# JaronTu/Multimodal_MVD_Seg

Hardware: AMD Instinct MI355X
Metric: train-step samples/sec on 4-modality 128^3 patches (PlainConvUNet 3d_fullres, fp32) (higher is better)
Workload: dtype f32; 1 GPU; BASELINE configs[1]: PlainConvUNet 3d_fullres 6 stages 31.2M params, 4x128x128x128 patch, 5 classes, fp32, DC+CE deep supervision, SGD-Nesterov+clip; per_gpu_batch=2, global_batch=2, parallelism=dp1, step_launch=one hipGraph replay per step (captured after 3 eager steps)

## Files before the change

include/mvdseg_hip.h:

```cpp
#ifndef MVDSEG_HIP_H
#define MVDSEG_HIP_H
#include <stddef.h>
#include <stdint.h>

#ifdef __cplusplus
extern "C" {
#endif

#define MVD_VERSION 100
#define MVD_MAX_TAPS 27

int mvd_version(void);
const char *mvd_last_error(void);
int mvd_has_mfma(void);
int mvd_set_conv_engine(int mode);
int mvd_set_wino_min_items(long n);

int mvd_pack_weight(const float *w, float *wf, float *wb, int K, int C, int T, int transposed, void *stream);

size_t mvd_conv_fwd_workspace_bytes(int N, long out_voxels, int K);
int mvd_conv3d_fwd(const float *x1, int C1, const float *x2, int C2, const float *wf, const float *bias, float *y,
                   int N, int D, int H, int W, int K, const int ksize[3], const int stride[3], void *ws,
                   size_t ws_bytes, void *stream);
int mvd_conv3d_dgrad(const float *dy, const float *wb, float *dx1, int C1, float *dx2, int C2, int N, int D, int H,
                     int W, int K, const int ksize[3], const int stride[3], void *ws, size_t ws_bytes, void *stream);
int mvd_conv_wino_applicable(int N, int D, int H, int W, int C1, int C2, int K, const int ksize[3], const int stride[3]);
size_t mvd_wino_weight_elems(int C, int K);
int mvd_wino_mode(void);
int mvd_pack_weight_wino(const float *w, float *uf, float *ub, int K, int C, void *stream);
int mvd_pack_weights_batch(int n, const float *const *w, float *const *wf, float *const *wb, float *const *uf,
                           float *const *ub, const int *K, const int *C, const int *T, const int *transposed,
                           void *stream);
int mvd_conv3d_fwd_wino(const float *x1, int C1, const float *x2, int C2, const float *wf, const float *uf,
                        const float *bias, float *y, int N, int D, int H, int W, int K, const int ksize[3],
                        const int stride[3], void *ws, size_t ws_bytes, void *stream);
size_t mvd_conv_stats_tiles(int D, int H, int W);
int mvd_conv3d_fwd_wino_stats(const float *x1, int C1, const float *x2, int C2, const float *wf, const float *uf,
                              const float *bias, float *y, float *stats, int *stats_done, int N, int D, int H, int W,
                              int K, const int ksize[3], const int stride[3], void *ws, size_t ws_bytes, void *stream);
int mvd_conv3d_dgrad_wino(const float *dy, const float *wb, const float *ub, float *dx1, int C1, float *dx2, int C2, int N,
                          int D, int H, int W, int K, const int ksize[3], const int stride[3], void *ws, size_t ws_bytes,
                          void *stream);
int mvd_set_wino3_min_items(long n);
int mvd_conv_wino3_applicable(int N, int D, int H, int W, int C1, int C2, int K, const int ksize[3], const int stride[3]);
size_t mvd_wino3_weight_elems(int C, int K);
int mvd_pack_weight_wino3(const float *w, float *vf, float *vb, int K, int C, void *stream);
int mvd_pack_weights_batch3(int n, const float *const *w, float *const *wf, float *const *wb, float *const *uf,
                            float *const *ub, float *const *vf, float *const *vb, const int *K, const int *C,
                            const int *T, const int *transposed, void *stream);
int mvd_conv3d_fwd_wino3(const float *x1, int C1, const float *x2, int C2, const float *wf, const float *vf,
                         const float *bias, float *y, int N, int D, int H, int W, int K, const int ksize[3],
                         const int stride[3], void *ws, size_t ws_bytes, void *stream);
int mvd_conv3d_fwd_wino3_stats(const float *x1, int C1, const float *x2, int C2, const float *wf, const float *vf,
                               const float *bias, float *y, float *stats, int *stats_done, int N, int D, int H, int W,
                               int K, const int ksize[3], const int stride[3], void *ws, size_t ws_bytes, void *stream);
int mvd_conv3d_dgrad_wino3(const float *dy, const float *wb, const float *vb, float *dx1, int C1, float *dx2, int C2,
                           int N, int D, int H, int W, int K, const int ksize[3], const int stride[3], void *ws,
                           size_t ws_bytes, void *stream);
int mvd_set_wgrad_wino3_min_items(long n);
int mvd_conv_wgrad_wino3_applicable(int N, int D, int H, int W, int C1, int C2, int K, const int ksize[3],
                                    const int stride[3]);
long mvd_wgrad_wino3_launches(void);
size_t mvd_conv3d_wgrad_workspace_bytes(int C, int K, int T, int N, int Do, int Ho, int Wo);
int mvd_conv3d_wgrad(const float *x1, int C1, const float *x2, int C2, const float *dy, float *dw, float *dbias,
                     int N, int D, int H, int W, int K, const int ksize[3], const int stride[3], void *ws,
                     size_t ws_bytes, void *stream);

int mvd_convT3d_fwd(const float *x, const float *wf, const float *bias, float *y, int N, int D, int H, int W, int C,
                    int K, const int stride[3], void *ws, size_t ws_bytes, void *stream);
int mvd_convT3d_dgrad(const float *dy, const float *wb, float *dx, int N, int D, int H, int W, int C, int K,
                      const int stride[3], void *ws, size_t ws_bytes, void *stream);
size_t mvd_convT3d_wgrad_workspace_bytes(int C, int K, int T, int N, int D, int H, int W);
int mvd_convT3d_wgrad(const float *x, const float *dy, float *dw, float *dbias, int N, int D, int H, int W, int C,
                      int K, const int stride[3], void *ws, size_t ws_bytes, void *stream);

int mvd_pack_weight_bf16(const float *w, uint16_t *wf, uint16_t *wb, int K, int C, int T, int transposed, void *stream);
int mvd_pack_weights_bf16_batch(int n, const float *const *w, uint16_t *const *wf, uint16_t *const *wb, const int *K,
                                const int *C, const int *T, const int *transposed, void *stream);
int mvd_pack_weights_bf16_batch_pad(int n, const float *const *w, uint16_t *const *wf, uint16_t *const *wb, const int *K,
                                    const int *C, const int *T, const int *transposed, const int *Csrc, void *stream);
int mvd_conv3d_fwd_bf16(const uint16_t *x1, int C1, const uint16_t *x2, int C2, const uint16_t *wf, const float *bias,
                        uint16_t *y, int N, int D, int H, int W, int K, const int ksize[3], const int stride[3],
                        void *ws, size_t ws_bytes, void *stream);
int mvd_conv3d_dgrad_bf16(const uint16_t *dy, const uint16_t *wb, uint16_t *dx1, int C1, uint16_t *dx2, int C2, int N,
                          int D, int H, int W, int K, const int ksize[3], const int stride[3], void *ws, size_t ws_bytes,
                          void *stream);
int mvd_convT3d_fwd_bf16(const uint16_t *x, const uint16_t *wf, const float *bias, uint16_t *y, int N, int D, int H, int W,
                         int C, int K, const int stride[3], void *ws, size_t ws_bytes, void *stream);
int mvd_convT3d_dgrad_bf16(const uint16_t *dy, const uint16_t *wb, uint16_t *dx, int N, int D, int H, int W, int C, int K,
                           const int stride[3], void *ws, size_t ws_bytes, void *stream);
int mvd_conv3d_wgrad_bf16(const uint16_t *x1, int C1, const uint16_t *x2, int C2, const uint16_t *dy, float *dw,
                          float *dbias, int N, int D, int H, int W, int K, const int ksize[3], const int stride[3],
                          void *ws, size_t ws_bytes, void *stream);
int mvd_convT3d_wgrad_bf16(const uint16_t *x, const uint16_t *dy, float *dw, float *dbias, int N, int D, int H, int W,
                           int C, int K, const int stride[3], void *ws, size_t ws_bytes, void *stream);
int mvd_conv3d_fwd_bf16_stats_tiles(int N, int D, int H, int W, int C1, int C2, int K, const int ksize[3],
                                    const int stride[3]);
int mvd_conv3d_dgrad_acc_ok(int is_bf16, int N, int D, int H, int W, int C1, int K, const int ksize[3], const int stride[3]);
int mvd_conv3d_dgrad_acc(const float *dy, const float *wb, float *dx1, int C1, int N, int D, int H, int W, int K,
                         const int ksize[3], const int stride[3], void *stream);
int mvd_conv3d_dgrad_bf16_acc(const uint16_t *dy, const uint16_t *wb, uint16_t *dx1, int C1, int N, int D, int H, int W, int K,
                              const int ksize[3], const int stride[3], void *ws, size_t ws_bytes, void *stream);
int mvd_set_bf16_zmarch_kernel(int which);
int mvd_set_bf16_wgrad_kernel(int which);
int mvd_conv3d_wgrad_bf16_prologue_ok(int N, int D, int H, int W, int C1, int C2, int K, const int ksize[3], const int stride[3]);
int mvd_conv3d_wgrad_bf16_fused(const uint16_t *x1, int C1, const uint16_t *dy, float *dw, float *dbias, int N, int D, int H, int W,
                                int K, const int ksize[3], const int stride[3], const float *in_scale, const float *in_shift,
                                float slope, void *ws, size_t ws_bytes, void *stream);
int mvd_conv3d_fwd_bf16_prologue_ok(int N, int D, int H, int W, int C1, int C2, int K, const int ksize[3],
                                    const int stride[3]);
int mvd_conv3d_fwd_bf16_fused(const uint16_t *x1, int C1, const uint16_t *x2, int C2, const uint16_t *wf, const float *bias,
                              uint16_t *y, int N, int D, int H, int W, int K, const int ksize[3], const int stride[3],
                              const float *in_scale, const float *in_shift, float slope, float *tile_stats, int *ntiles_out,
                              void *ws, size_t ws_bytes, void *stream);
int mvd_instnorm_finalize_tiles(const float *tile_stats, long ntiles, const float *gamma, const float *beta, float *mean,
                                float *rstd, float *scale, float *shift, int N, long V, int C, float eps, void *stream);
int mvd_instnorm_lrelu_apply_bf16(const uint16_t *x, const float *scale, const float *shift, uint16_t *y, int N, long V,
                                  int C, float slope, void *stream);
int mvd_instnorm_stats_bf16(const void *x, int x_is_bf16, const float *gamma, const float *beta, float *mean, float *rstd,
                            float *scale, float *shift, int N, long V, int C, float eps, void *ws, size_t ws_bytes,
                            void *stream);
int mvd_instnorm_lrelu_fwd_bf16(const void *x, int x_is_bf16, const float *gamma, const float *beta, uint16_t *y,
                                float *mean, float *rstd, int N, long V, int C, float eps, float slope, void *ws,
                                size_t ws_bytes, void *stream);
int mvd_instnorm_lrelu_bwd_bf16(const void *x, int x_is_bf16, const uint16_t *dy, const float *gamma, const float *beta,
                                const float *mean, const float *rstd, void *dx, float *dgamma, float *dbeta, int N,
                                long V, int C, float slope, void *ws, size_t ws_bytes, void *stream);
int mvd_seghead_fwd_bf16(const uint16_t *x, const float *w, const float *bias, float *logits, int N, long V, int C,
                         int K, void *stream);
int mvd_seghead_bwd_bf16(const uint16_t *x, const float *w, const float *dlogits, uint16_t *dx, float *dw, float *dbias,
                         int N, long V, int C, int K, int accumulate, void *ws, size_t ws_bytes, void *stream);
int mvd_seghead_bf16_fused_ok(int N, long V, int C, int K);
int mvd_seghead_fwd_fused(const float *x, const float *mean, const float *rstd, const float *gamma, const float *beta, float slope,
                          const float *w, const float *bias, float *logits, int N, long V, int C, int K, void *stream);
int mvd_seghead_bwd_fused(const float *x, const float *mean, const float *rstd, const float *gamma, const float *beta, float slope,
                          const float *w, const float *dlogits, float *dx, float *dw, float *dbias, int N, long V, int C, int K,
                          int accumulate, void *ws, size_t ws_bytes, void *stream);
int mvd_instnorm_stats_from_tiles(const float *tile_stats, long ntiles, float *mean, float *rstd, int N, long V, int C, float eps,
                                  void *ws, size_t ws_bytes, void *stream);
int mvd_seghead_fwd_bf16_fused(const uint16_t *x, const float *scale, const float *shift, float slope, const float *w,
                               const float *bias, float *logits, int N, long V, int C, int K, void *stream);
int mvd_seghead_bwd_bf16_fused(const uint16_t *x, const float *scale, const float *shift, float slope, const float *w,
                               const float *dlogits, uint16_t *dx, float *dw, float *dbias, int N, long V, int C, int K,
                               int accumulate, void *ws, size_t ws_bytes, void *stream);
int mvd_cast_f32_to_bf16(const float *src, uint16_t *dst, long n, void *stream);
int mvd_cast_bf16_to_f32(const uint16_t *src, float *dst, long n, void *stream);

int mvd_instnorm_nblk(int N, long V, int C);
size_t mvd_instnorm_workspace_bytes(int N, long V, int C);
int mvd_instnorm_lrelu_fwd(const float *x, const float *gamma, const float *beta, float *y, float *mean,
                           float *rstd, int N, long V, int C, float eps, float slope, void *ws, size_t ws_bytes,
                           void *stream);
int mvd_instnorm_lrelu_fwd_prestats(const float *x, const float *tile_stats, long ntiles, const float *gamma,
                                    const float *beta, float *y, float *mean, float *rstd, int N, long V, int C, float eps,
                                    float slope, void *ws, size_t ws_bytes, void *stream);
int mvd_instnorm_lrelu_bwd(const float *x, const float *dy, const float *gamma, const float *beta,
                           const float *mean, const float *rstd, float *dx, float *dgamma, float *dbeta, int N,
                           long V, int C, float slope, void *ws, size_t ws_bytes, void *stream);

int mvd_seghead_fwd(const float *x, const float *w, const float *bias, float *logits, int N, long V, int C, int K,
                    void *stream);
size_t mvd_seghead_bwd_workspace_bytes(int N, long V, int C, int K);
int mvd_seghead_bwd(const float *x, const float *w, const float *dlogits, float *dx, float *dw, float *dbias, int N,
                    long V, int C, int K, int accumulate, void *ws, size_t ws_bytes, void *stream);

size_t mvd_dcce_workspace_bytes(int N, long V, int K);
int mvd_dcce_fwd(const float *logits, const float *target, float *stats , int N, long V, int K, void *ws,
                 size_t ws_bytes, void *stream);
int mvd_dcce_finalize(const float *stats, int N, const float *dstats, int Nd, float *loss, float *coef, long V, int K,
                      int batch_dice, int do_bg, float smooth, float w_ce, float w_dice, void *stream);
int mvd_dcce_bwd(const float *logits, const float *target, const float *coef , const float *gscale_dev,
                 float gscale_host, float *dlogits, int N, long V, int K, float w_ce, void *stream);
int mvd_softmax_select_fwd(const float *logits, float *p_sel, int N, long V, int K, int sel, void *stream);
int mvd_softmax_select_bwd(const float *logits, const float *g, float *dlogits, int N, long V, int K, int sel,
                           void *stream);
int mvd_label_mask(const float *labels, float *mask, long n, float value, void *stream);
int mvd_argmax_counts(const float *logits, const float *target, long long *counts, int N, long V, int K,
                      void *stream);

size_t mvd_kl_workspace_bytes(int N, long V);
int mvd_kl_fwd(const float *ys, const float *yt, float *out, int N, int C, long V, long sn, long sc, long sv,
               float T, float eps_s, int pad_zero_channel, void *ws, size_t ws_bytes, void *stream);
int mvd_kl_bwd(const float *ys, const float *yt, const float *gscale_dev, float gscale_host, float *gs, float *gt,
               int N, int C, long V, long sn, long sc, long sv, float T, float eps_s, int pad_zero_channel,
               void *stream);
// ... 141 lines not shown
```

multimodal_mvd_seg_amd/_lib.py:

```python
import ctypes
import os
from ctypes import c_float, c_int, c_long, c_size_t, c_uint64, c_void_p

_HERE = os.path.dirname(os.path.abspath(__file__))
LIB_PATH = os.path.join(_HERE, "libmvdseg_hip.so")

_P = c_void_p
_I3 = ctypes.c_int * 3

SIGNATURES = {
    "mvd_version": (c_int, []),
    "mvd_last_error": (ctypes.c_char_p, []),
    "mvd_has_mfma": (c_int, []),
    "mvd_set_conv_engine": (c_int, [c_int]),
    "mvd_set_wino_min_items": (c_int, [c_long]),
    "mvd_pack_weight": (c_int, [_P, _P, _P, c_int, c_int, c_int, c_int, _P]),
    "mvd_conv_fwd_workspace_bytes": (c_size_t, [c_int, c_long, c_int]),
    "mvd_conv3d_fwd": (c_int, [_P, c_int, _P, c_int, _P, _P, _P, c_int, c_int, c_int, c_int, c_int, _I3, _I3, _P,
                               c_size_t, _P]),
    "mvd_conv3d_dgrad": (c_int, [_P, _P, _P, c_int, _P, c_int, c_int, c_int, c_int, c_int, c_int, _I3, _I3, _P,
                                 c_size_t, _P]),
    "mvd_conv3d_wgrad_workspace_bytes": (c_size_t, [c_int, c_int, c_int, c_int, c_int, c_int, c_int]),
    "mvd_conv3d_wgrad": (c_int, [_P, c_int, _P, c_int, _P, _P, _P, c_int, c_int, c_int, c_int, c_int, _I3, _I3, _P,
                                 c_size_t, _P]),
    "mvd_convT3d_fwd": (c_int, [_P, _P, _P, _P, c_int, c_int, c_int, c_int, c_int, c_int, _I3, _P, c_size_t, _P]),
    "mvd_convT3d_dgrad": (c_int, [_P, _P, _P, c_int, c_int, c_int, c_int, c_int, c_int, _I3, _P, c_size_t, _P]),
    "mvd_convT3d_wgrad_workspace_bytes": (c_size_t, [c_int, c_int, c_int, c_int, c_int, c_int, c_int]),
    "mvd_convT3d_wgrad": (c_int, [_P, _P, _P, _P, c_int, c_int, c_int, c_int, c_int, c_int, _I3, _P, c_size_t, _P]),
    "mvd_conv_wino_applicable": (c_int, [c_int, c_int, c_int, c_int, c_int, c_int, c_int, _I3, _I3]),
    "mvd_wino_mode": (c_int, []),
    "mvd_wino_weight_elems": (c_size_t, [c_int, c_int]),
    "mvd_pack_weight_wino": (c_int, [_P, _P, _P, c_int, c_int, _P]),
    "mvd_pack_weights_batch": (c_int, [c_int] + [_P] * 9 + [_P]),
    "mvd_conv3d_fwd_wino": (c_int, [_P, c_int, _P, c_int, _P, _P, _P, _P, c_int, c_int, c_int, c_int, c_int, _I3, _I3, _P,
                                    c_size_t, _P]),
    "mvd_conv_stats_tiles": (c_size_t, [c_int, c_int, c_int]),
    "mvd_conv3d_fwd_wino_stats": (c_int, [_P, c_int, _P, c_int, _P, _P, _P, _P, _P, _P, c_int, c_int, c_int, c_int, c_int,
                                          _I3, _I3, _P, c_size_t, _P]),
    "mvd_conv3d_dgrad_wino": (c_int, [_P, _P, _P, _P, c_int, _P, c_int, c_int, c_int, c_int, c_int, c_int, _I3, _I3, _P,
                                      c_size_t, _P]),
    "mvd_set_wino3_min_items": (c_int, [c_long]),
    "mvd_conv_wino3_applicable": (c_int, [c_int, c_int, c_int, c_int, c_int, c_int, c_int, _I3, _I3]),
    "mvd_wino3_weight_elems": (c_size_t, [c_int, c_int]),
    "mvd_pack_weight_wino3": (c_int, [_P, _P, _P, c_int, c_int, _P]),
    "mvd_pack_weights_batch3": (c_int, [c_int] + [_P] * 11 + [_P]),
    "mvd_conv3d_fwd_wino3": (c_int, [_P, c_int, _P, c_int, _P, _P, _P, _P, c_int, c_int, c_int, c_int, c_int, _I3, _I3, _P,
                                     c_size_t, _P]),
    "mvd_conv3d_fwd_wino3_stats": (c_int, [_P, c_int, _P, c_int, _P, _P, _P, _P, _P, _P, c_int, c_int, c_int, c_int, c_int,
                                           _I3, _I3, _P, c_size_t, _P]),
    "mvd_conv3d_dgrad_wino3": (c_int, [_P, _P, _P, _P, c_int, _P, c_int, c_int, c_int, c_int, c_int, c_int, _I3, _I3, _P,
                                       c_size_t, _P]),
    "mvd_set_wgrad_wino3_min_items": (c_int, [c_long]),
    "mvd_conv_wgrad_wino3_applicable": (c_int, [c_int, c_int, c_int, c_int, c_int, c_int, c_int, _I3, _I3]),
    "mvd_wgrad_wino3_launches": (c_long, []),
    "mvd_conv3d_wgrad_bf16": (c_int, [_P, c_int, _P, c_int, _P, _P, _P, c_int, c_int, c_int, c_int, c_int, _I3, _I3, _P,
                                      c_size_t, _P]),
    "mvd_convT3d_wgrad_bf16": (c_int, [_P, _P, _P, _P, c_int, c_int, c_int, c_int, c_int, c_int, _I3, _P, c_size_t,
                                       _P]),
    "mvd_instnorm_lrelu_fwd_prestats": (c_int, [_P, _P, c_long, _P, _P, _P, _P, _P, c_int, c_long, c_int, c_float, c_float,
                                                _P, c_size_t, _P]),
    "mvd_conv3d_fwd_bf16_stats_tiles": (c_int, [c_int, c_int, c_int, c_int, c_int, c_int, c_int, _I3, _I3]),
    "mvd_set_bf16_zmarch_kernel": (c_int, [c_int]),
    "mvd_set_bf16_wgrad_kernel": (c_int, [c_int]),
    "mvd_conv3d_dgrad_acc_ok": (c_int, [c_int, c_int, c_int, c_int, c_int, c_int, c_int, _I3, _I3]),
    "mvd_conv3d_dgrad_acc": (c_int, [_P, _P, _P, c_int, c_int, c_int, c_int, c_int, c_int, _I3, _I3, _P]),
    "mvd_conv3d_dgrad_bf16_acc": (c_int, [_P, _P, _P, c_int, c_int, c_int, c_int, c_int, c_int, _I3, _I3, _P, c_size_t, _P]),
    "mvd_conv3d_fwd_bf16_prologue_ok": (c_int, [c_int, c_int, c_int, c_int, c_int, c_int, c_int, _I3, _I3]),
    "mvd_conv3d_wgrad_bf16_prologue_ok": (c_int, [c_int, c_int, c_int, c_int, c_int, c_int, c_int, _I3, _I3]),
    "mvd_conv3d_wgrad_bf16_fused": (c_int, [_P, c_int, _P, _P, _P, c_int, c_int, c_int, c_int, c_int, _I3, _I3, _P, _P, c_float,
                                            _P, c_size_t, _P]),
    "mvd_instnorm_stats_bf16": (c_int, [_P, c_int, _P, _P, _P, _P, _P, _P, c_int, c_long, c_int, c_float, _P, c_size_t, _P]),
    "mvd_conv3d_fwd_bf16_fused": (c_int, [_P, c_int, _P, c_int, _P, _P, _P, c_int, c_int, c_int, c_int, c_int, _I3, _I3, _P,
                                          _P, c_float, _P, _P, _P, c_size_t, _P]),
    "mvd_instnorm_finalize_tiles": (c_int, [_P, c_long, _P, _P, _P, _P, _P, _P, c_int, c_long, c_int, c_float, _P]),
    "mvd_instnorm_lrelu_apply_bf16": (c_int, [_P, _P, _P, _P, c_int, c_long, c_int, c_float, _P]),
    "mvd_instnorm_lrelu_fwd_bf16": (c_int, [_P, c_int, _P, _P, _P, _P, _P, c_int, c_long, c_int, c_float, c_float, _P,
                                            c_size_t, _P]),
    "mvd_instnorm_lrelu_bwd_bf16": (c_int, [_P, c_int, _P, _P, _P, _P, _P, _P, _P, _P, c_int, c_long, c_int, c_float, _P,
                                            c_size_t, _P]),
    "mvd_seghead_fwd_bf16": (c_int, [_P, _P, _P, _P, c_int, c_long, c_int, c_int, _P]),
    "mvd_seghead_bwd_bf16": (c_int, [_P, _P, _P, _P, _P, _P, c_int, c_long, c_int, c_int, c_int, _P, c_size_t, _P]),
    "mvd_seghead_bf16_fused_ok": (c_int, [c_int, c_long, c_int, c_int]),
    "mvd_seghead_fwd_fused": (c_int, [_P, _P, _P, _P, _P, c_float, _P, _P, _P, c_int, c_long, c_int, c_int, _P]),
    "mvd_seghead_bwd_fused": (c_int, [_P, _P, _P, _P, _P, c_float, _P, _P, _P, _P, _P, c_int, c_long, c_int, c_int, c_int, _P,
                                      c_size_t, _P]),
    "mvd_instnorm_stats_from_tiles": (c_int, [_P, c_long, _P, _P, c_int, c_long, c_int, c_float, _P, c_size_t, _P]),
    "mvd_seghead_fwd_bf16_fused": (c_int, [_P, _P, _P, c_float, _P, _P, _P, c_int, c_long, c_int, c_int, _P]),
    "mvd_seghead_bwd_bf16_fused": (c_int, [_P, _P, _P, c_float, _P, _P, _P, _P, _P, c_int, c_long, c_int, c_int, c_int, _P,
                                           c_size_t, _P]),
    "mvd_cast_f32_to_bf16": (c_int, [_P, _P, c_long, _P]),
    "mvd_cast_bf16_to_f32": (c_int, [_P, _P, c_long, _P]),
    "mvd_pack_weight_bf16": (c_int, [_P, _P, _P, c_int, c_int, c_int, c_int, _P]),
    "mvd_pack_weights_bf16_batch": (c_int, [c_int] + [_P] * 7 + [_P]),
    "mvd_pack_weights_bf16_batch_pad": (c_int, [c_int] + [_P] * 8 + [_P]),
    "mvd_conv3d_fwd_bf16": (c_int, [_P, c_int, _P, c_int, _P, _P, _P, c_int, c_int, c_int, c_int, c_int, _I3, _I3, _P,
                                    c_size_t, _P]),
    "mvd_conv3d_dgrad_bf16": (c_int, [_P, _P, _P, c_int, _P, c_int, c_int, c_int, c_int, c_int, c_int, _I3, _I3, _P,
                                      c_size_t, _P]),
    "mvd_convT3d_fwd_bf16": (c_int, [_P, _P, _P, _P, c_int, c_int, c_int, c_int, c_int, c_int, _I3, _P, c_size_t, _P]),
    "mvd_convT3d_dgrad_bf16": (c_int, [_P, _P, _P, c_int, c_int, c_int, c_int, c_int, c_int, _I3, _P, c_size_t, _P]),
    "mvd_instnorm_nblk": (c_int, [c_int, c_long, c_int]),
    "mvd_instnorm_workspace_bytes": (c_size_t, [c_int, c_long, c_int]),
    "mvd_instnorm_lrelu_fwd": (c_int, [_P, _P, _P, _P, _P, _P, c_int, c_long, c_int, c_float, c_float, _P, c_size_t, _P]),
    "mvd_instnorm_lrelu_bwd": (c_int, [_P, _P, _P, _P, _P, _P, _P, _P, _P, c_int, c_long, c_int, c_float, _P, c_size_t,
                                       _P]),
    "mvd_seghead_fwd": (c_int, [_P, _P, _P, _P, c_int, c_long, c_int, c_int, _P]),
    "mvd_seghead_bwd_workspace_bytes": (c_size_t, [c_int, c_long, c_int, c_int]),
    "mvd_seghead_bwd": (c_int, [_P, _P, _P, _P, _P, _P, c_int, c_long, c_int, c_int, c_int, _P, c_size_t, _P]),
    "mvd_dcce_workspace_bytes": (c_size_t, [c_int, c_long, c_int]),
    "mvd_dcce_fwd": (c_int, [_P, _P, _P, c_int, c_long, c_int, _P, c_size_t, _P]),
    "mvd_dcce_finalize": (c_int, [_P, c_int, _P, c_int, _P, _P, c_long, c_int, c_int, c_int, c_float, c_float, c_float,
                                  _P]),
    "mvd_dcce_bwd": (c_int, [_P, _P, _P, _P, c_float, _P, c_int, c_long, c_int, c_float, _P]),
    "mvd_argmax_counts": (c_int, [_P, _P, _P, c_int, c_long, c_int, _P]),
    "mvd_softmax_select_fwd": (c_int, [_P, _P, c_int, c_long, c_int, c_int, _P]),
    "mvd_softmax_select_bwd": (c_int, [_P, _P, _P, c_int, c_long, c_int, c_int, _P]),
    "mvd_label_mask": (c_int, [_P, _P, c_long, c_float, _P]),
    "mvd_cldice_combine": (c_int, [_P, _P, c_float, _P]),
    "mvd_kl_workspace_bytes": (c_size_t, [c_int, c_long]),
    "mvd_kl_fwd": (c_int, [_P, _P, _P, c_int, c_int, c_long, c_long, c_long, c_long, c_float, c_float, c_int, _P,
                           c_size_t, _P]),
    "mvd_kl_bwd": (c_int, [_P, _P, _P, c_float, _P, _P, c_int, c_int, c_long, c_long, c_long, c_long, c_float, c_float,
                           c_int, _P]),
    "mvd_kl_fwd_bf16": (c_int, [_P, _P, _P, c_int, c_int, c_long, c_float, c_float, _P, c_size_t, _P]),
    "mvd_kl_bwd_bf16": (c_int, [_P, _P, _P, c_float, _P, _P, c_int, c_int, c_long, c_float, c_float, _P]),
    "mvd_mse_workspace_bytes": (c_size_t, [c_long]),
    "mvd_mse_fwd": (c_int, [_P, _P, _P, c_long, _P, c_size_t, _P]),
    "mvd_mse_bwd": (c_int, [_P, _P, _P, _P, _P, c_long, _P]),
    "mvd_soft_erode_fwd": (c_int, [_P, _P, _P, c_int, c_int, c_int, c_int, _P]),
    "mvd_soft_erode_bwd": (c_int, [_P, _P, _P, c_int, c_int, c_int, c_int, _P]),
    "mvd_soft_dilate_fwd": (c_int, [_P, _P, _P, c_int, c_int, c_int, c_int, _P]),
    "mvd_soft_dilate_bwd": (c_int, [_P, _P, _P, c_int, c_int, c_int, c_int, _P]),
    "mvd_skel_update_fwd": (c_int, [_P, _P, _P, _P, c_long, c_int, _P]),
    "mvd_skel_update_bwd": (c_int, [_P, _P, _P, _P, _P, _P, _P, c_long, c_int, _P]),
# ... 99 lines not shown
```

multimodal_mvd_seg_amd/csrc/conv.hip:

```cpp
#include "common.h"
#include "conv_geom.h"

namespace mvd {

static int g_engine_mode = 0;
#define g_wino_off (wino_mode() == 0)
static const int g_transp_off = getenv("MVD_TRANSP") ? (atoi(getenv("MVD_TRANSP")) == 0) : 0;
static long g_wino_min_items = getenv("MVD_WINO_MIN") ? atol(getenv("MVD_WINO_MIN")) : 256;
static const long kWino3MinItemsDefault = 128;
static long g_wino3_min_items = getenv("MVD_WINO3_MIN") ? atol(getenv("MVD_WINO3_MIN")) : kWino3MinItemsDefault;
static long wino3_items(int D, int H, int W, int K) { return (long)((D + 3) / 4) * ((H + 7) / 8) * ((W + 7) / 8) * (K / 32); }

__global__ void k_fwd_scalar(FwdGeom g, const float *__restrict__ a1, const float *__restrict__ a2,
                             const float *__restrict__ w, const float *__restrict__ bias, float *__restrict__ y1,
                             float *__restrict__ y2) {
    const int K = g.K1 + g.K2, C = g.C1 + g.C2;
    const int CK = wl_ck(C);
    const long total = (long)g.N * g.Do * g.Ho * g.Wo * K;
    for (long idx = (long)blockIdx.x * blockDim.x + threadIdx.x; idx < total; idx += (long)gridDim.x * blockDim.x) {
        int k = (int)(idx % K);
        long r = idx / K;
        int ow = (int)(r % g.Wo);
        r /= g.Wo;
        int oh = (int)(r % g.Ho);
// ... 185 lines not shown
        partial[(size_t)blockIdx.x * K + k] = s;
    }
}

static int colsum_blocks(long rows, long *chunk) {
    long nb = rows / 256;
    if (nb < 1) nb = 1;
    if (nb > 2048) nb = 2048;
    *chunk = cdiv(rows, nb);
    return (int)cdiv(rows, *chunk);
}
static size_t colsum_ws(long rows, int K) {
    long chunk;
    return (size_t)colsum_blocks(rows, &chunk) * K * sizeof(double) + 256;
}
static int colsum(const float *x, float *out, long rows, int K, void *ws, hipStream_t s, bool bf = false) {
    long chunk;
    int nb = colsum_blocks(rows, &chunk);
    double *partial = reinterpret_cast<double *>(ws);
    if (K % 4 == 0 && K <= 1024 && (((uintptr_t)x) & 15) == 0) {
        const int KG = K / 4;
        const int R = 256 / KG > 0 ? 256 / KG : 1;
        const int threads = (R * KG + 63) / 64 * 64;
        if (bf)
            hipLaunchKernelGGL(k_colsum4<true>, dim3(nb), dim3(threads), (size_t)R * K * sizeof(double), s, x, partial, rows,
                               K, chunk);
        else
            hipLaunchKernelGGL(k_colsum4<false>, dim3(nb), dim3(threads), (size_t)R * K * sizeof(double), s, x, partial, rows,
                               K, chunk);
    } else if (bf) {
        set_error("bias grad (bf16): K %% 4 != 0 is not supported");
        return 2;
    } else {
        hipLaunchKernelGGL(k_colsum, dim3(nb), dim3(256), 0, s, x, partial, rows, K, chunk);
    }
    if (check_launch("bias grad")) return 1;
    return reduce_partials(partial, out, nb, K, s);
}

static inline int out_dim(int in, int k, int s) { return (in + 2 * ((k - 1) / 2) - k) / s + 1; }

static int check_ks(const int ks[3], const int st[3], const char *who) {
    for (int a = 0; a < 3; a++) {
        if (!(ks[a] == 1 || ks[a] == 3)) {
            set_error("%s: kernel size must be 1 or 3 per axis (got %d)", who, ks[a]);
            return 1;
        }
        if (!(st[a] == 1 || st[a] == 2)) {
            set_error("%s: stride must be 1 or 2 per axis (got %d)", who, st[a]);
            return 1;
        }
    }
    return 0;
}

static void conv_fwd_geom(FwdGeom &g, int N, int D, int H, int W, int C1, int C2, int K, const int ks[3],
                          const int st[3]) {
    memset(&g, 0, sizeof(g));
    g.N = N;
    g.Di = D; g.Hi = H; g.Wi = W;
    g.Do = out_dim(D, ks[0], st[0]); g.Ho = out_dim(H, ks[1], st[1]); g.Wo = out_dim(W, ks[2], st[2]);
    g.Dy = g.Do; g.Hy = g.Ho; g.Wy = g.Wo;
    g.C1 = C1; g.C2 = C2; g.K1 = K; g.K2 = 0;
    int t = 0;
    for (int a = 0; a < ks[0]; a++)
        for (int b = 0; b < ks[1]; b++)
            for (int c = 0; c < ks[2]; c++) {
                g.off[t][0] = a - (ks[0] - 1) / 2;
                g.off[t][1] = b - (ks[1] - 1) / 2;
                g.off[t][2] = c - (ks[2] - 1) / 2;
                g.wt[t] = t;
                t++;
            }
    g.ntaps = g.T = t;
    for (int a = 0; a < 3; a++) {
        g.sa[a] = st[a];
        g.so[a] = 1;
        g.oo[a] = 0;
    }
}

static int run_fwd(const FwdGeom &g, const float *a1, const float *a2, const float *w, const float *bias, float *y1,
                   float *y2, void *ws, size_t ws_bytes, hipStream_t s, const float *u = nullptr, float *stats = nullptr,
                   int *stats_done = nullptr, bool u3d = false) {
    if (stats_done) *stats_done = 0;
    if (u3d) {
        if (g_engine_mode == 0 && u && !g_wino_off && wino3_enabled() &&
            wino3_items(g.Do, g.Ho, g.Wo, g.K1 + g.K2) >= g_wino3_min_items) {
            int r = fwd_wino3(g, a1, a2, u, bias, y1, y2, s, stats, stats_done);
            if (r >= 0) return r;
            if (stats_done) *stats_done = 0;
        }
        u = nullptr;
    }
    if (g_engine_mode == 0 && u && !g_wino_off) {
        const long tiles = (long)g.N * ((g.Do + 3) / 4) * ((g.Ho + 3) / 4) * ((g.Wo + 7) / 8) * ((g.K1 + g.K2) / 32);
        if (tiles >= g_wino_min_items) {
            int r = fwd_wino(g, a1, a2, u, bias, y1, y2, s, stats, stats_done);
            if (r >= 0) return r;
            if (stats_done) *stats_done = 0;
        }
    }
    if (g_engine_mode == 0) {
        int r = fwd_mfma(g, a1, a2, w, bias, y1, y2, ws, ws_bytes, s);
        if (r >= 0) return r;
    }
    return fwd_scalar(g, a1, a2, w, bias, y1, y2, s);
}

static int run_wgrad(const WgradGeom &g, const float *a1, const float *a2, const float *b, float *dw, void *ws,
                     size_t ws_bytes, hipStream_t s, float *dbias = nullptr, int *dbias_done = nullptr) {
    if (dbias_done) *dbias_done = 0;
    if (g_engine_mode == 0) {
        int r = wgrad_mfma(g, a1, a2, b, dw, ws, ws_bytes, s, false, dbias, dbias_done);
        if (r >= 0) return r;
        if (dbias_done) *dbias_done = 0;
    }
    return wgrad_scalar(g, a1, a2, b, dw, ws, ws_bytes, s);
}

static int run_fwd16(const FwdGeom &g, const uint16_t *a1, const uint16_t *a2, const uint16_t *w, const float *bias,
                     uint16_t *y1, uint16_t *y2, void *ws, size_t ws_bytes, hipStream_t s, const Fwd16Fuse *fuse = nullptr) {
    int r = fwd_bf16(g, a1, a2, w, bias, y1, y2, ws, ws_bytes, s, fuse);
    if (r < 0 && fuse && fuse->in_scale) {
        set_error("bf16 conv engine: the fused InstanceNorm input prologue needs the z-marching kernel (3x3x3 stride 1, 32 -> 32 "
                  "channels, >= 4 tiles per CU); C=%d+%d K=%d+%d", g.C1, g.C2, g.K1, g.K2);
        return 3;
    }
    if (r < 0) {
        set_error("bf16 conv engine: unsupported shape (needs C %% 32 == 0 and K %% 32 == 0; C=%d+%d K=%d+%d)", g.C1, g.C2,
                  g.K1, g.K2);
        return 3;
    }
    return r;
}

static int run_wgrad16(const WgradGeom &g, const uint16_t *a1, const uint16_t *a2, const uint16_t *b, float *dw, void *ws,
                       size_t ws_bytes, hipStream_t s, float *dbias = nullptr, int *dbias_done = nullptr) {
    int r = wgrad_mfma(g, reinterpret_cast<const float *>(a1), reinterpret_cast<const float *>(a2),
                       reinterpret_cast<const float *>(b), dw, ws, ws_bytes, s, true, dbias, dbias_done);
    if (r < 0) {
        set_error("bf16 wgrad: unsupported shape (needs C %% 32 == 0 and K %% 32 == 0; C=%d+%d K=%d)", g.C1, g.C2, g.K);
        return 3;
    }
    return r;
}

static size_t max_sz(size_t a, size_t b) { return a > b ? a : b; }

}

using namespace mvd;

extern "C" {

int mvd_set_conv_engine(int mode) {
    g_engine_mode = mode ? 1 : 0;
    return 0;
}

int mvd_set_wino_min_items(long n) {
    g_wino_min_items = n < 0 ? 256 : n;
    return 0;
}

size_t mvd_conv_fwd_workspace_bytes(int N, long out_voxels, int K) { return fwd_mfma_ws(N, out_voxels, K); }

static int conv3d_fwd_impl(const float *x1, int C1, const float *x2, int C2, const float *wf, const float *uf,
                           const float *bias, float *y, int N, int D, int H, int W, int K, const int ksize[3],
                           const int stride[3], void *ws, size_t ws_bytes, void *stream, float *stats = nullptr,
                           int *stats_done = nullptr, bool u3d = false) {
    MVD_REQUIRE(x1 && wf && y && C1 > 0 && C2 >= 0 && (C2 == 0 || x2), "conv3d_fwd: null pointer / bad channels");
// ... 35 lines not shown
                              const float *bias, float *y, float *stats, int *stats_done, int N, int D, int H, int W,
                              int K, const int ksize[3], const int stride[3], void *ws, size_t ws_bytes, void *stream) {
    MVD_REQUIRE(stats_done, "conv3d_fwd_wino_stats: stats_done is required");
    return conv3d_fwd_impl(x1, C1, x2, C2, wf, uf, bias, y, N, D, H, W, K, ksize, stride, ws, ws_bytes, stream, stats,
                           stats_done);
}

int mvd_pack_weights_batch(int n, const float *const *w, float *const *wf, float *const *wb, float *const *uf,
                           float *const *ub, const int *K, const int *C, const int *T, const int *transposed,
                           void *stream) {
    MVD_REQUIRE(n > 0 && w && wf && wb && uf && ub && K && C && T && transposed, "pack_weights_batch: null table");
    for (int q = 0; q < n; q++) {
        MVD_REQUIRE(w[q] && (wf[q] || wb[q] || uf[q] || ub[q]), "pack_weights_batch: job without source or destination");
        MVD_REQUIRE(K[q] > 0 && C[q] > 0 && T[q] > 0 && T[q] <= MVD_MAX_TAPS, "pack_weights_batch: bad K / C / T");
        if (uf[q] || ub[q]) {
            MVD_REQUIRE(wino_mode() == 2, "pack_weights_batch: Winograd tables need MVD_WINO=2 (F(2x2,3x3) layout)");
            MVD_REQUIRE(T[q] == 27 && !transposed[q] && K[q] % 32 == 0 && C[q] % 32 == 0,
                        "pack_weights_batch: Winograd tables need a 3x3x3 conv with C %% 32 == 0 and K %% 32 == 0");
        }
    }
    return pack_weights_batch(n, w, wf, wb, uf, ub, K, C, T, transposed, as_stream(stream));
}

int mvd_pack_weight_wino(const float *w, float *uf, float *ub, int K, int C, void *stream) {
    MVD_REQUIRE(w && (uf || ub) && K > 0 && C > 0, "pack_weight_wino: bad arguments");
    MVD_REQUIRE(K % 32 == 0 && C % 32 == 0, "pack_weight_wino: needs C %% 32 == 0 and K %% 32 == 0");
    return pack_weight_wino(w, uf, ub, K, C, as_stream(stream));
}

int mvd_set_wino3_min_items(long n) {
    g_wino3_min_items = n < 0 ? kWino3MinItemsDefault : n;
    return 0;
}

int mvd_conv_wino3_applicable(int N, int D, int H, int W, int C1, int C2, int K, const int ksize[3], const int stride[3]) {
    if (!wino3_enabled()) return 0;
    const int two = mvd_conv_wino_applicable(N, D, H, W, C1, C2, K, ksize, stride);
    return two & ((wino3_items(D, H, W, K) >= g_wino3_min_items ? 1 : 0) |
                  (wino3_items(D, H, W, C1 + C2) >= g_wino3_min_items ? 2 : 0));
}

size_t mvd_wino3_weight_elems(int C, int K) { return (size_t)64 * C * K; }

int mvd_pack_weight_wino3(const float *w, float *uf, float *ub, int K, int C, void *stream) {
    MVD_REQUIRE(w && (uf || ub) && K > 0 && C > 0, "pack_weight_wino3: bad arguments");
    MVD_REQUIRE(K % 32 == 0 && C % 32 == 0, "pack_weight_wino3: needs C %% 32 == 0 and K %% 32 == 0");
    return pack_weight_wino3(w, uf, ub, K, C, as_stream(stream));
}

int mvd_pack_weights_batch3(int n, const float *const *w, float *const *wf, float *const *wb, float *const *uf,
                            float *const *ub, float *const *vf, float *const *vb, const int *K, const int *C,
                            const int *T, const int *transposed, void *stream) {
    MVD_REQUIRE(n > 0 && w && wf && wb && uf && ub && vf && vb && K && C && T && transposed,
                "pack_weights_batch3: null table");
    for (int q = 0; q < n; q++) {
        MVD_REQUIRE(w[q] && (wf[q] || wb[q] || uf[q] || ub[q] || vf[q] || vb[q]),
                    "pack_weights_batch3: job without source or destination");
        MVD_REQUIRE(K[q] > 0 && C[q] > 0 && T[q] > 0 && T[q] <= MVD_MAX_TAPS, "pack_weights_batch3: bad K / C / T");
        if (uf[q] || ub[q]) MVD_REQUIRE(wino_mode() == 2, "pack_weights_batch3: Winograd tables need MVD_WINO=2");
        if (uf[q] || ub[q] || vf[q] || vb[q])
            MVD_REQUIRE(T[q] == 27 && !transposed[q] && K[q] % 32 == 0 && C[q] % 32 == 0,
                        "pack_weights_batch3: Winograd tables need a 3x3x3 conv with C %% 32 == 0 and K %% 32 == 0");
    }
    return pack_weights_batch(n, w, wf, wb, uf, ub, K, C, T, transposed, as_stream(stream), vf, vb);
}

int mvd_conv3d_fwd_wino3(const float *x1, int C1, const float *x2, int C2, const float *wf, const float *vf,
                         const float *bias, float *y, int N, int D, int H, int W, int K, const int ksize[3],
                         const int stride[3], void *ws, size_t ws_bytes, void *stream) {
    return conv3d_fwd_impl(x1, C1, x2, C2, wf, vf, bias, y, N, D, H, W, K, ksize, stride, ws, ws_bytes, stream, nullptr,
                           nullptr, true);
}

int mvd_conv3d_fwd_wino3_stats(const float *x1, int C1, const float *x2, int C2, const float *wf, const float *vf,
                               const float *bias, float *y, float *stats, int *stats_done, int N, int D, int H, int W,
                               int K, const int ksize[3], const int stride[3], void *ws, size_t ws_bytes, void *stream) {
    MVD_REQUIRE(stats_done, "conv3d_fwd_wino3_stats: stats_done is required");
    return conv3d_fwd_impl(x1, C1, x2, C2, wf, vf, bias, y, N, D, H, W, K, ksize, stride, ws, ws_bytes, stream, stats,
                           stats_done, true);
}

static int conv3d_dgrad_impl(const float *dy, const float *wb, const float *ub, float *dx1, int C1, float *dx2, int C2,
                             int N, int D, int H, int W, int K, const int ksize[3], const int stride[3], void *ws,
                             size_t ws_bytes, void *stream, bool u3d = false);

int mvd_conv3d_dgrad(const float *dy, const float *wb, float *dx1, int C1, float *dx2, int C2, int N, int D, int H, int W,
                     int K, const int ksize[3], const int stride[3], void *ws, size_t ws_bytes, void *stream) {
    return conv3d_dgrad_impl(dy, wb, nullptr, dx1, C1, dx2, C2, N, D, H, W, K, ksize, stride, ws, ws_bytes, stream);
}

int mvd_conv3d_dgrad_wino(const float *dy, const float *wb, const float *ub, float *dx1, int C1, float *dx2, int C2, int N,
                          int D, int H, int W, int K, const int ksize[3], const int stride[3], void *ws, size_t ws_bytes,
                          void *stream) {
    return conv3d_dgrad_impl(dy, wb, ub, dx1, C1, dx2, C2, N, D, H, W, K, ksize, stride, ws, ws_bytes, stream);
}

int mvd_conv3d_dgrad_wino3(const float *dy, const float *wb, const float *vb, float *dx1, int C1, float *dx2, int C2,
                           int N, int D, int H, int W, int K, const int ksize[3], const int stride[3], void *ws,
                           size_t ws_bytes, void *stream) {
    return conv3d_dgrad_impl(dy, wb, vb, dx1, C1, dx2, C2, N, D, H, W, K, ksize, stride, ws, ws_bytes, stream, true);
}

static int conv3d_dgrad_impl(const float *dy, const float *wb, const float *ub, float *dx1, int C1, float *dx2, int C2,
                             int N, int D, int H, int W, int K, const int ksize[3], const int stride[3], void *ws,
                             size_t ws_bytes, void *stream, bool u3d) {
    MVD_REQUIRE(dy && wb && dx1 && C1 > 0 && C2 >= 0 && (C2 == 0 || dx2), "conv3d_dgrad: null pointer / bad channels");
    MVD_REQUIRE(N > 0 && D > 0 && H > 0 && W > 0 && K > 0, "conv3d_dgrad: bad shape");
    if (check_ks(ksize, stride, "conv3d_dgrad")) return 2;
    const int dims[3] = {D, H, W};
    int od[3], pad[3];
    for (int a = 0; a < 3; a++) {
        od[a] = out_dim(dims[a], ksize[a], stride[a]);
        pad[a] = (ksize[a] - 1) / 2;
    }
    static int dg2 = -1;
    if (dg2 < 0) dg2 = getenv("MVD_DGRAD2") ? atoi(getenv("MVD_DGRAD2")) : 1;
    if (dg2 && g_engine_mode == 0 && C2 == 0 && ksize[0] == 3 && ksize[1] == 3 && ksize[2] == 3 && stride[0] == 2 &&
        stride[1] == 2 && stride[2] == 2 && ((long)N * od[0] * od[1] * od[2] >= 4096 || g_wino_min_items <= 1)) {
        int r = dgrad32s(N, D, H, W, C1, K, od[0], od[1], od[2], dy, wb, dx1, as_stream(stream));
        if (r >= 0) return r;
    }
    for (int pd = 0; pd < stride[0]; pd++)
        for (int ph = 0; ph < stride[1]; ph++)
            for (int pw = 0; pw < stride[2]; pw++) {
                const int p[3] = {pd, ph, pw};
                FwdGeom g;
                memset(&g, 0, sizeof(g));
                g.N = N;
                g.Di = od[0]; g.Hi = od[1]; g.Wi = od[2];
                g.Dy = D; g.Hy = H; g.Wy = W;
                int grid[3];
                bool empty = false;
                for (int a = 0; a < 3; a++) {
                    grid[a] = (dims[a] - p[a] + stride[a] - 1) / stride[a];
                    if (grid[a] <= 0) empty = true;
                    g.sa[a] = 1;
                    g.so[a] = stride[a];
                    g.oo[a] = p[a];
                }
                if (empty) continue;
                g.Do = grid[0]; g.Ho = grid[1]; g.Wo = grid[2];
                g.C1 = K; g.C2 = 0; g.K1 = C1; g.K2 = C2;
                int nt = 0;
                for (int ta = 0; ta < ksize[0]; ta++)
                    for (int tb = 0; tb < ksize[1]; tb++)
                        for (int tc = 0; tc < ksize[2]; tc++) {
                            const int t3[3] = {ta, tb, tc};
                            int off[3];
                            bool ok = true;
                            for (int a = 0; a < 3; a++) {
                                int num = p[a] + pad[a] - t3[a];
                                if (num % stride[a] != 0) { ok = false; break; }
                                off[a] = num / stride[a];
                            }
                            if (!ok) continue;
                            for (int a = 0; a < 3; a++) g.off[nt][a] = (int8_t)off[a];
                            g.wt[nt] = (int8_t)((ta * ksize[1] + tb) * ksize[2] + tc);
                            nt++;
                        }
                g.ntaps = nt;
                g.T = ksize[0] * ksize[1] * ksize[2];
                if (nt == 0) continue;
                int r = run_fwd(g, dy, nullptr, wb, nullptr, dx1, dx2, ws, ws_bytes, as_stream(stream), ub, nullptr, nullptr,
                                u3d);
                if (r) return r;
            }
    return 0;
}

static void conv_wgrad_geom(WgradGeom &g, int N, int D, int H, int W, int C1, int C2, int K, const int ks[3],
                            const int st[3]) {
    memset(&g, 0, sizeof(g));
    g.N = N;
    g.Di = D; g.Hi = H; g.Wi = W;
    g.Do = out_dim(D, ks[0], st[0]); g.Ho = out_dim(H, ks[1], st[1]); g.Wo = out_dim(W, ks[2], st[2]);
    g.Db = g.Do; g.Hb = g.Ho; g.Wb = g.Wo;
    g.C1 = C1; g.C2 = C2; g.K = K;
    int t = 0;
    for (int a = 0; a < ks[0]; a++)
        for (int b = 0; b < ks[1]; b++)
            for (int c = 0; c < ks[2]; c++) {
                g.off[t][0] = a - (ks[0] - 1) / 2;
                g.off[t][1] = b - (ks[1] - 1) / 2;
                g.off[t][2] = c - (ks[2] - 1) / 2;
                g.wt[t] = t;
                t++;
            }
    g.ntaps = g.T = t;
    for (int a = 0; a < 3; a++) {
        g.sa[a] = st[a];
        g.sb[a] = 1;
    }
    g.transposed_out = 0;
}

size_t mvd_conv3d_wgrad_workspace_bytes(int C, int K, int T, int N, int Do, int Ho, int Wo) {
    WgradGeom g;
    memset(&g, 0, sizeof(g));
    g.N = N; g.Do = Do; g.Ho = Ho; g.Wo = Wo; g.C1 = C; g.C2 = 0; g.K = K; g.ntaps = g.T = T;
    size_t a = max_sz(wgrad_scalar_ws(g), wgrad_mfma_ws(g));
    return max_sz(a, colsum_ws((long)N * Do * Ho * Wo, K));
}

int mvd_set_wgrad_wino3_min_items(long n) {
    set_wgrad_wino3_min_items(n);
    return 0;
}

int mvd_conv_wgrad_wino3_applicable(int N, int D, int H, int W, int C1, int C2, int K, const int ksize[3],
                                    const int stride[3]) {
    if (N <= 0 || D <= 0 || H <= 0 || W <= 0 || C1 <= 0 || C2 < 0 || K <= 0 || !ksize || !stride) return 0;
    for (int a = 0; a < 3; a++)
        if (ksize[a] != 3 || stride[a] != 1) return 0;
    WgradGeom g;
    conv_wgrad_geom(g, N, D, H, W, C1, C2, K, ksize, stride);
    return wgrad_wino3_selected(g) ? 1 : 0;
}

long mvd_wgrad_wino3_launches(void) { return wgrad_wino3_launches(); }

int mvd_conv3d_wgrad(const float *x1, int C1, const float *x2, int C2, const float *dy, float *dw, float *dbias, int N,
                     int D, int H, int W, int K, const int ksize[3], const int stride[3], void *ws, size_t ws_bytes,
                     void *stream) {
    MVD_REQUIRE(x1 && dy && dw && ws && C1 > 0 && C2 >= 0 && (C2 == 0 || x2), "conv3d_wgrad: null pointer / bad channels");
    MVD_REQUIRE(N > 0 && D > 0 && H > 0 && W > 0 && K > 0, "conv3d_wgrad: bad shape");
    if (check_ks(ksize, stride, "conv3d_wgrad")) return 2;
    WgradGeom g;
    conv_wgrad_geom(g, N, D, H, W, C1, C2, K, ksize, stride);
    MVD_REQUIRE(ws_bytes >= mvd_conv3d_wgrad_workspace_bytes(C1 + C2, K, g.T, N, g.Do, g.Ho, g.Wo),
                "conv3d_wgrad: workspace too small");
    hipStream_t s = as_stream(stream);
    int dbias_done = 0;
    int r = run_wgrad(g, x1, x2, dy, dw, ws, ws_bytes, s, dbias, &dbias_done);
    if (r) return r;
    if (dbias && !dbias_done) return colsum(dy, dbias, (long)N * g.Do * g.Ho * g.Wo, K, ws, s);
    return 0;
}

int mvd_convT3d_fwd(const float *x, const float *wf, const float *bias, float *y, int N, int D, int H, int W, int C, int K,
                    const int stride[3], void *ws, size_t ws_bytes, void *stream) {
    MVD_REQUIRE(x && wf && y && N > 0 && D > 0 && H > 0 && W > 0 && C > 0 && K > 0, "convT3d_fwd: bad arguments");
    for (int a = 0; a < 3; a++) MVD_REQUIRE(stride[a] == 1 || stride[a] == 2, "convT3d_fwd: stride must be 1 or 2");
    if (g_engine_mode == 0 && !g_transp_off) {
        int r = convT_fwd_direct(x, wf, bias, y, N, D, H, W, C, K, stride, as_stream(stream));
        if (r >= 0) return r;
    }
    for (int pd = 0; pd < stride[0]; pd++)
// ... 224 lines not shown
                memset(&g, 0, sizeof(g));
                g.N = N;
                g.Di = od[0]; g.Hi = od[1]; g.Wi = od[2];
                g.Dy = D; g.Hy = H; g.Wy = W;
                int grid[3];
                bool empty = false;
                for (int a = 0; a < 3; a++) {
                    grid[a] = (dims[a] - p[a] + stride[a] - 1) / stride[a];
                    if (grid[a] <= 0) empty = true;
                    g.sa[a] = 1;
                    g.so[a] = stride[a];
                    g.oo[a] = p[a];
                }
                if (empty) continue;
                g.Do = grid[0]; g.Ho = grid[1]; g.Wo = grid[2];
                g.C1 = K; g.C2 = 0; g.K1 = C1; g.K2 = C2;
                int nt = 0;
                for (int ta = 0; ta < ksize[0]; ta++)
                    for (int tb = 0; tb < ksize[1]; tb++)
                        for (int tc = 0; tc < ksize[2]; tc++) {
                            const int t3[3] = {ta, tb, tc};
                            int off[3];
                            bool ok = true;
                            for (int a = 0; a < 3; a++) {
                                int num = p[a] + pad[a] - t3[a];
                                if (num % stride[a] != 0) { ok = false; break; }
                                off[a] = num / stride[a];
                            }
                            if (!ok) continue;
                            for (int a = 0; a < 3; a++) g.off[nt][a] = (int8_t)off[a];
                            g.wt[nt] = (int8_t)((ta * ksize[1] + tb) * ksize[2] + tc);
                            nt++;
                        }
                g.ntaps = nt;
                g.T = ksize[0] * ksize[1] * ksize[2];
                g.acc = (int8_t)acc;
                if (nt == 0) continue;
                int r = run_fwd16(g, dy, nullptr, wb, nullptr, dx1, dx2, ws, ws_bytes, as_stream(stream));
                if (r) return r;
            }
    return 0;
}

int mvd_conv3d_dgrad_bf16(const uint16_t *dy, const uint16_t *wb, uint16_t *dx1, int C1, uint16_t *dx2, int C2, int N, int D, int H, int W,
                     int K, const int ksize[3], const int stride[3], void *ws, size_t ws_bytes, void *stream) {
    return dgrad_bf16_impl(dy, wb, dx1, C1, dx2, C2, N, D, H, W, K, ksize, stride, ws, ws_bytes, stream, 0);
}

static bool strided3(const int ksize[3], const int stride[3]) {
    return ksize[0] == 3 && ksize[1] == 3 && ksize[2] == 3 && (stride[0] == 2 || stride[1] == 2 || stride[2] == 2);
}

int mvd_conv3d_dgrad_acc_ok(int is_bf16, int N, int D, int H, int W, int C1, int K, const int ksize[3], const int stride[3]) {
    if (N <= 0 || D <= 0 || H <= 0 || W <= 0 || C1 <= 0 || K <= 0 || check_ks(ksize, stride, "conv3d_dgrad_acc_ok")) return 0;
    if (C1 % 32 || K % 32 || g_engine_mode != 0) return 0;
    if (is_bf16) return strided3(ksize, stride) ? 1 : 0;
    if (!(ksize[0] == 3 && ksize[1] == 3 && ksize[2] == 3 && stride[0] == 2 && stride[1] == 2 && stride[2] == 2)) return 0;
    const long items = (long)N * out_dim(D, 3, 2) * out_dim(H, 3, 2) * out_dim(W, 3, 2);
    static int dg2 = -1;
    if (dg2 < 0) dg2 = getenv("MVD_DGRAD2") ? atoi(getenv("MVD_DGRAD2")) : 1;
    return (dg2 && (items >= 4096 || g_wino_min_items <= 1) && (long)out_dim(D, 3, 2) * out_dim(H, 3, 2) * out_dim(W, 3, 2) * K * 4 < (1L << 31)) ? 1 : 0;
}

int mvd_conv3d_dgrad_bf16_acc(const uint16_t *dy, const uint16_t *wb, uint16_t *dx1, int C1, int N, int D, int H, int W, int K,
                              const int ksize[3], const int stride[3], void *ws, size_t ws_bytes, void *stream) {
    MVD_REQUIRE(mvd_conv3d_dgrad_acc_ok(1, N, D, H, W, C1, K, ksize, stride), "conv3d_dgrad_bf16_acc: no accumulating kernel for this "
                "shape (ask mvd_conv3d_dgrad_acc_ok first)");
    return dgrad_bf16_impl(dy, wb, dx1, C1, nullptr, 0, N, D, H, W, K, ksize, stride, ws, ws_bytes, stream, 1);
}

int mvd_conv3d_dgrad_acc(const float *dy, const float *wb, float *dx1, int C1, int N, int D, int H, int W, int K,
                         const int ksize[3], const int stride[3], void *stream) {
    MVD_REQUIRE(dy && wb && dx1, "conv3d_dgrad_acc: null pointer");
    MVD_REQUIRE(mvd_conv3d_dgrad_acc_ok(0, N, D, H, W, C1, K, ksize, stride), "conv3d_dgrad_acc: no accumulating kernel for this shape "
                "(ask mvd_conv3d_dgrad_acc_ok first)");
    int r = dgrad32s(N, D, H, W, C1, K, out_dim(D, 3, 2), out_dim(H, 3, 2), out_dim(W, 3, 2), dy, wb, dx1, as_stream(stream), 1);
    if (r < 0) {
        set_error("conv3d_dgrad_acc: the fused stride-2 kernel refused the shape");
        return 3;
    }
    return r;
}

int mvd_convT3d_fwd_bf16(const uint16_t *x, const uint16_t *wf, const float *bias, uint16_t *y, int N, int D, int H, int W, int C, int K,
                    const int stride[3], void *ws, size_t ws_bytes, void *stream) {
    MVD_REQUIRE(x && wf && y && N > 0 && D > 0 && H > 0 && W > 0 && C > 0 && K > 0, "convT3d_fwd_bf16: bad arguments");
    for (int a = 0; a < 3; a++) MVD_REQUIRE(stride[a] == 1 || stride[a] == 2, "convT3d_fwd_bf16: stride must be 1 or 2");
    if (!g_transp_off) {
        int r = convT_fwd_direct16(x, wf, bias, y, N, D, H, W, C, K, stride, as_stream(stream));
        if (r >= 0) return r;
    }
    for (int pd = 0; pd < stride[0]; pd++)
        for (int ph = 0; ph < stride[1]; ph++)
            for (int pw = 0; pw < stride[2]; pw++) {
                FwdGeom g;
                memset(&g, 0, sizeof(g));
                g.N = N;
                g.Di = g.Do = D; g.Hi = g.Ho = H; g.Wi = g.Wo = W;
                g.Dy = D * stride[0]; g.Hy = H * stride[1]; g.Wy = W * stride[2];
                g.C1 = C; g.K1 = K;
                g.ntaps = 1;
                g.T = stride[0] * stride[1] * stride[2];
                g.wt[0] = (int8_t)((pd * stride[1] + ph) * stride[2] + pw);
                const int p[3] = {pd, ph, pw};
                for (int a = 0; a < 3; a++) {
                    g.sa[a] = 1;
                    g.so[a] = stride[a];
                    g.oo[a] = p[a];
                }
                int r = run_fwd16(g, x, nullptr, wf, bias, y, nullptr, ws, ws_bytes, as_stream(stream));
                if (r) return r;
            }
    return 0;
}

int mvd_convT3d_dgrad_bf16(const uint16_t *dy, const uint16_t *wb, uint16_t *dx, int N, int D, int H, int W, int C, int K,
                      const int stride[3], void *ws, size_t ws_bytes, void *stream) {
    MVD_REQUIRE(dy && wb && dx && N > 0 && D > 0 && H > 0 && W > 0 && C > 0 && K > 0, "convT3d_dgrad_bf16: bad arguments");
    for (int a = 0; a < 3; a++) MVD_REQUIRE(stride[a] == 1 || stride[a] == 2, "convT3d_dgrad_bf16: stride must be 1 or 2");
    if (!g_transp_off) {
        int r = convT_dgrad_direct16(dy, wb, dx, N, D, H, W, C, K, stride, as_stream(stream));
        if (r >= 0) return r;
    }
    FwdGeom g;
    memset(&g, 0, sizeof(g));
    g.N = N;
    g.Di = D * stride[0]; g.Hi = H * stride[1]; g.Wi = W * stride[2];
    g.Do = g.Dy = D; g.Ho = g.Hy = H; g.Wo = g.Wy = W;
    g.C1 = K; g.K1 = C;
    int t = 0;
    for (int pd = 0; pd < stride[0]; pd++)
        for (int ph = 0; ph < stride[1]; ph++)
            for (int pw = 0; pw < stride[2]; pw++) {
                g.off[t][0] = pd; g.off[t][1] = ph; g.off[t][2] = pw;
                g.wt[t] = t;
                t++;
            }
    g.ntaps = g.T = t;
    for (int a = 0; a < 3; a++) {
        g.sa[a] = stride[a];
        g.so[a] = 1;
        g.oo[a] = 0;
    }
    return run_fwd16(g, dy, nullptr, wb, nullptr, dx, nullptr, ws, ws_bytes, as_stream(stream));
}

int mvd_conv3d_wgrad_bf16(const uint16_t *x1, int C1, const uint16_t *x2, int C2, const uint16_t *dy, float *dw, float *dbias, int N,
                     int D, int H, int W, int K, const int ksize[3], const int stride[3], void *ws, size_t ws_bytes,
                     void *stream) {
    MVD_REQUIRE(x1 && dy && dw && ws && C1 > 0 && C2 >= 0 && (C2 == 0 || x2), "conv3d_wgrad_bf16: null pointer / bad channels");
    MVD_REQUIRE(N > 0 && D > 0 && H > 0 && W > 0 && K > 0, "conv3d_wgrad_bf16: bad shape");
    if (check_ks(ksize, stride, "conv3d_wgrad_bf16")) return 2;
    WgradGeom g;
    conv_wgrad_geom(g, N, D, H, W, C1, C2, K, ksize, stride);
    MVD_REQUIRE(ws_bytes >= mvd_conv3d_wgrad_workspace_bytes(C1 + C2, K, g.T, N, g.Do, g.Ho, g.Wo),
                "conv3d_wgrad_bf16: workspace too small");
    hipStream_t s = as_stream(stream);
    int dbias_done = 0;
    int r = run_wgrad16(g, x1, x2, dy, dw, ws, ws_bytes, s, dbias, &dbias_done);
    if (r) return r;
    if (dbias && !dbias_done) return colsum(reinterpret_cast<const float *>(dy), dbias, (long)N * g.Do * g.Ho * g.Wo, K, ws, s, true);
    return 0;
}

int mvd_conv3d_wgrad_bf16_prologue_ok(int N, int D, int H, int W, int C1, int C2, int K, const int ksize[3], const int stride[3]) {
    if (N <= 0 || D <= 0 || H <= 0 || W <= 0 || C1 <= 0 || C2 < 0 || K <= 0 || check_ks(ksize, stride, "conv3d_wgrad_bf16_prologue_ok"))
// ... 45 lines not shown
```

multimodal_mvd_seg_amd/csrc/conv_geom.h:

```cpp
#pragma once
#include <stdint.h>

namespace mvd {

__host__ __device__ inline int wl_ck(int C) {
    return (C % 32 == 0) ? 32 : ((C % 8 == 0) ? 8 : ((C % 4 == 0) ? 4 : 0));
}
__host__ __device__ inline size_t widx(int CK, int T, int C, int K, int t, int c, int k) {
    if (CK == 0) return ((size_t)t * C + c) * K + k;
    const int hh = CK / 2;
    const int cc = c / CK, r = c % CK;
    return ((((size_t)cc * T + t) * 2 + r / hh) * K + k) * hh + (r % hh);
}

struct FwdGeom {
    int N;
    int T;
    int Di, Hi, Wi;
    int Do, Ho, Wo;
    int Dy, Hy, Wy;
    int C1, C2, K1, K2;
    int ntaps;
    int sa[3], so[3], oo[3];
    int8_t off[27][3];
    int8_t wt[27];
    int8_t acc;
};

struct WgradGeom {
    int N;
    int Di, Hi, Wi;
    int Db, Hb, Wb;
    int Do, Ho, Wo;
    int C1, C2, K;
    int ntaps;
    int T;
    int sa[3], sb[3];
    int8_t off[27][3], ob[27][3];
    int8_t wt[27];
    int transposed_out;
};

int fwd_scalar(const FwdGeom &g, const float *a1, const float *a2, const float *w, const float *bias, float *y1,
               float *y2, hipStream_t s);
size_t fwd_mfma_ws(int N, long out_vox, int K);
int fwd_mfma(const FwdGeom &g, const float *a1, const float *a2, const float *w, const float *bias, float *y1, float *y2,
             void *ws, size_t ws_bytes, hipStream_t s);
size_t wgrad_scalar_ws(const WgradGeom &g);
int wgrad_scalar(const WgradGeom &g, const float *a1, const float *a2, const float *b, float *dw, void *ws,
                 size_t ws_bytes, hipStream_t s);
size_t wgrad_mfma_ws(const WgradGeom &g);
int wgrad_mfma(const WgradGeom &g, const float *a1, const float *a2, const float *b, float *dw, void *ws, size_t ws_bytes,
               hipStream_t s, bool bf16_in = false, float *dbias = nullptr, int *dbias_done = nullptr);

int fwd_wino(const FwdGeom &g, const float *a1, const float *a2, const float *u, const float *bias, float *y1, float *y2,
             hipStream_t s, float *stats = nullptr, int *stats_done = nullptr);
int pack_weight_wino(const float *w, float *uf, float *ub, int K, int C, hipStream_t s);
int fwd_wino3(const FwdGeom &g, const float *a1, const float *a2, const float *u, const float *bias, float *y1, float *y2,
              hipStream_t s, float *stats = nullptr, int *stats_done = nullptr);
int pack_weight_wino3(const float *w, float *uf, float *ub, int K, int C, hipStream_t s);
int wino3_enabled();
int dgrad32s(int N, int D, int H, int W, int C, int K, int Do, int Ho, int Wo, const float *dy, const float *wb, float *dx,
             hipStream_t s, int accumulate = 0);
int dgrad16s(int N, int D, int H, int W, int C, int K, int Do, int Ho, int Wo, const unsigned short *dy, const unsigned short *wb,
             unsigned short *dx, hipStream_t s, int accumulate = 0);
int launch_fwd16ys(const FwdGeom &g, const unsigned short *a1, const unsigned short *a2, const unsigned short *w, const float *bias,
                   unsigned short *y1, unsigned short *y2, hipStream_t s, int ncu);
int wgrad16z(const WgradGeom &g, const unsigned short *a1, const unsigned short *a2, const unsigned short *b, void *ws,
             size_t ws_bytes, bool want_bias, int *nsplit_out, float **pbias_out, hipStream_t s, const float *in_scale = nullptr,
             const float *in_shift = nullptr, float slope = 0.f);
int wgrad16z_run(const WgradGeom &g, const unsigned short *a1, const unsigned short *a2, const unsigned short *b, float *dw, void *ws,
                 size_t ws_bytes, hipStream_t s, float *dbias, int *dbias_done, const float *in_scale, const float *in_shift,
                 float slope);
bool wgrad16z_prologue_ok(const WgradGeom &g);
int wgrad16zs(const WgradGeom &g, const unsigned short *a1, const unsigned short *a2, const unsigned short *b, void *ws,
              size_t ws_bytes, int *nsplit_out, hipStream_t s);
void wgrad16z_enable(int on);
int pack_weights_batch(int n, const float *const *w, float *const *wf, float *const *wb, float *const *uf, float *const *ub,
                       const int *K, const int *C, const int *T, const int *transposed, hipStream_t s,
                       float *const *vf = nullptr, float *const *vb = nullptr);
int wino_mode();
int wgrad_wino3(const WgradGeom &g, const float *a1, const float *a2, const float *b, float *dw, void *ws, size_t ws_bytes,
                int nsplit, hipStream_t s, float *dbias, int *dbias_done);
bool wgrad_wino3_selected(const WgradGeom &g);
size_t wgrad_wino3_ws(int nsplit, int C, int K);
int wgrad_wino3_enabled();
void set_wgrad_wino3_min_items(long n);
long wgrad_wino3_launches();
int dbias_reduce(const float *pbias, float *dbias, int K, int nrows, hipStream_t s);
size_t wino_weight_elems(int C, int K);

int convT_fwd_direct(const float *x, const float *wf, const float *bias, float *y, int N, int D, int H, int W, int C, int K,
                     const int st[3], hipStream_t s);
int convT_dgrad_direct(const float *dy, const float *wb, float *dx, int N, int D, int H, int W, int C, int K,
                       const int st[3], hipStream_t s);

int convT_fwd_direct16(const unsigned short *x, const unsigned short *wf, const float *bias, unsigned short *y, int N, int D,
                       int H, int W, int C, int K, const int st[3], hipStream_t s);
int convT_dgrad_direct16(const unsigned short *dy, const unsigned short *wb, unsigned short *dx, int N, int D, int H, int W,
                         int C, int K, const int st[3], hipStream_t s);

struct Fwd16Fuse {
    float *tile_stats = nullptr;
    int *ntiles = nullptr;
    const float *in_scale = nullptr, *in_shift = nullptr;
    float slope = 0.01f;
};
int fwd_bf16(const FwdGeom &g, const unsigned short *a1, const unsigned short *a2, const unsigned short *w,
             const float *bias, unsigned short *y1, unsigned short *y2, void *ws, size_t ws_bytes, hipStream_t s,
             const Fwd16Fuse *fuse = nullptr);
int fwd16y_enabled();
void fwd16y_enable(int on);
int launch_fwd16y(const FwdGeom &g, const unsigned short *a1, const unsigned short *a2, const unsigned short *w,
                  const float *bias, unsigned short *y1, unsigned short *y2, hipStream_t s, const Fwd16Fuse *fuse, int ncu,
                  int *stats_tiles_only);
int fwd_bf16_stats_tiles(const FwdGeom &g);
int fwd_bf16_prologue_ok(const FwdGeom &g);
int pack_weight16(const float *w, unsigned short *wf, unsigned short *wb, int K, int C, int T, int transposed,
                  hipStream_t s);
int pack_weights16_batch(int n, const float *const *w, unsigned short *const *wf, unsigned short *const *wb, const int *K,
                         const int *C, const int *T, const int *transposed, const int *Csrc, hipStream_t s);

}
```

multimodal_mvd_seg_amd/csrc/conv_mfma.hip:

```cpp
#include <stdlib.h>
#include <type_traits>

#include "common.h"
#include "conv_geom.h"

namespace mvd {

typedef float f32x16 __attribute__((ext_vector_type(16)));

struct FwdTile {
    int ED, EH, EW, nslots;
    int min_off[3];
    int ntd, nth, ntw;
    int K;
    int toff[27];
    int dbg;
};

__device__ __forceinline__ void store_tile32(const FwdGeom &g, const f32x16 &acc, float bv, int n, int od, int ohb, int ow0,
                                             int k, int hh, int S, int split, int Ktot, float *__restrict__ part,
                                             float *__restrict__ y1, float *__restrict__ y2) {
    const int owl = ow0 + 4 * hh;
    if (S > 1) {
        float *pl = part + (size_t)(4 * hh) * Ktot + k;
// ... 519 lines not shown
                        const int ez = slot / EHW, rem2 = slot - ez * EHW;
                        const int ey = (rem2 * tg.magW) >> 16, ex = rem2 - ey * tg.EW;
                        const int id = iz0 + ez, ih = iy0 + ey, iw2 = ix0 + ex;
                        if (id >= 0 && id < g.Di && ih >= 0 && ih < g.Hi && iw2 >= 0 && iw2 < g.Wi)
                            v[q] = *reinterpret_cast<const float4 *>(
                                src + ((((size_t)n * g.Di + id) * g.Hi + ih) * g.Wi + iw2) * Cs + cofs + (tid_ & 7) * 4);
                    }
                }
#pragma unroll
                for (int q = 0; q < SXB; q++) {
                    const int idx = (base + q) * 512 + tid_;
                    if (idx < nx) *reinterpret_cast<float4 *>(Xs + (size_t)(idx >> 3) * XS + (idx & 7) * 4) = v[q];
                }
            }
        }
        __syncthreads();
        float4 af[2][4];
        {
            const float4 *pa = xlane + (size_t)__builtin_amdgcn_readlane(toff_l, tb) * (XS / 4);
#pragma unroll
            for (int e = 0; e < 4; e++) af[0][e] = pa[e];
        }
        for (int s0 = 0; s0 < nt; s0 += 4) {
#pragma unroll
            for (int u = 0; u < 4; u++) {
                const int sidx = s0 + u;
                if (sidx < nt) {
                    const int t = tb + sidx;
                    const int tn = sidx + 3 < nt ? t + 3 : tb + nt - 1;
#pragma unroll
                    for (int e = 0; e < 4; e++)
                        wb[(u + 3) & 3][e] =
                            *reinterpret_cast<const float4 *>(wc + (size_t)__builtin_amdgcn_readlane(wt_l, tn) * wtap + e * 4);
                    const float4 *pa = xlane + (size_t)__builtin_amdgcn_readlane(toff_l, sidx + 1 < nt ? t + 1 : tb + nt - 1) * (XS / 4);
#pragma unroll
                    for (int e = 0; e < 4; e++) af[(u + 1) & 1][e] = pa[e];
#pragma unroll
                    for (int e = 0; e < 4; e++) {
                        acc = __builtin_amdgcn_mfma_f32_32x32x2f32(af[u & 1][e].x, wb[u][e].x, acc, 0, 0, 0);
                        acc = __builtin_amdgcn_mfma_f32_32x32x2f32(af[u & 1][e].y, wb[u][e].y, acc, 0, 0, 0);
                        acc = __builtin_amdgcn_mfma_f32_32x32x2f32(af[u & 1][e].z, wb[u][e].z, acc, 0, 0, 0);
                        acc = __builtin_amdgcn_mfma_f32_32x32x2f32(af[u & 1][e].w, wb[u][e].w, acc, 0, 0, 0);
                    }
                    __builtin_amdgcn_sched_barrier(0);
                }
            }
        }
    }
    __syncthreads();
    if (tap_half) {
        float *xo = Xs + (size_t)(wave & 3) * 1024 + lane;
#pragma unroll
        for (int r = 0; r < 16; r++) xo[r * 64] = acc[r];
    }
    __syncthreads();
    if (tap_half) return;
    {
        const float *xi = Xs + (size_t)wave * 1024 + lane;
#pragma unroll
        for (int r = 0; r < 16; r++) acc[r] += xi[r * 64];
    }
    const int od = od0 + dl;
    if (od >= g.Do) return;
    const float bv = settled(bias ? bias[kcol] : 0.f);
#pragma unroll
    for (int r = 0; r < 16; r++) {
        const int row = (r & 3) + 8 * (r >> 2) + 4 * h;
        const int oh = oh0 + (row >> 3), ow = ow0 + (row & 7);
        if (oh < g.Ho && ow < g.Wo) {
            const size_t ov = (((size_t)n * g.Dy + od) * g.Hy + oh) * g.Wy + ow;
            const float val = acc[r] + bv;
            if (kcol < g.K1)
                y1[ov * g.K1 + kcol] = val;
            else
                y2[ov * g.K2 + (kcol - g.K1)] = val;
        }
    }
}

struct Dg2Tile {
    int ntd, nth, ntw, ncb, nitems, C;
    int acc;
};
__global__ __launch_bounds__(512, 2) void k_dgrad32s(const FwdGeom g, const Dg2Tile tg, const float *__restrict__ dy,
                                                     const float *__restrict__ wb, float *__restrict__ dx) {
    __shared__ __attribute__((aligned(16))) float Xs[135 * 36];
    constexpr int XS = 36;
    const int tid = threadIdx.x, lane = tid & 63;
    const int wave = __builtin_amdgcn_readfirstlane(tid >> 6);
    const int i = lane & 31, h = lane >> 5;
    const int per_xcd = (tg.nitems + 7) >> 3;
    const int item = (int)(blockIdx.x & 7) * per_xcd + (int)(blockIdx.x >> 3);
    if (item >= tg.nitems) return;
    unsigned r_ = (unsigned)item;
    const int cb = (int)(r_ % (unsigned)tg.ncb); r_ /= (unsigned)tg.ncb;
    const int tw_ = (int)(r_ % (unsigned)tg.ntw); r_ /= (unsigned)tg.ntw;
    const int th_ = (int)(r_ % (unsigned)tg.nth); r_ /= (unsigned)tg.nth;
    const int td_ = (int)(r_ % (unsigned)tg.ntd);
    const int n = (int)(r_ / (unsigned)tg.ntd);
    const int K = g.C1, C = tg.C;
    const int nch = K >> 5;
    const int oz0 = td_ * 2, oy0 = th_ * 4, ox0 = tw_ * 8;
    const int ccol = cb * 32 + i;
    const float *wlane = wb + (((size_t)h * C + ccol) << 4);
    const size_t wtap = (size_t)2 * C * 16;

    f32x16 acc[2];
#pragma unroll
    for (int m = 0; m < 2; m++)
#pragma unroll
        for (int r = 0; r < 16; r++) acc[m][r] = 0.f;

    for (int kk = 0; kk < nch; kk++) {
        __syncthreads();
        {
            const __amdgpu_buffer_rsrc_t rdy = __builtin_amdgcn_make_buffer_rsrc(
                const_cast<float *>(dy + (size_t)n * g.Di * g.Hi * g.Wi * K + kk * 32), 0, 0x7fffffff, 0x00020000);
            float4 v[3];
#pragma unroll
            for (int u = 0; u < 3; u++) {
                const int idx = tid + u * 512;
                const int slot = idx >> 3, part = idx & 7;
                const int ez = slot / 45, rem = slot - ez * 45;
                const int ey = rem / 9, ex = rem - ey * 9;
                const int oz = oz0 + ez, oy = oy0 + ey, ox = ox0 + ex;
                const bool ok = idx < 135 * 8 && oz < g.Di && oy < g.Hi && ox < g.Wi;
                const unsigned o = ok ? (unsigned)(((oz * g.Hi + oy) * g.Wi + ox) * K + part * 4) * 4u : 0xffffffffu;
                v[u] = __builtin_bit_cast(float4, __builtin_amdgcn_raw_buffer_load_b128(rdy, (int)o, 0, 0));
            }
#pragma unroll
            for (int u = 0; u < 3; u++) {
                const int idx = tid + u * 512;
                if (idx < 135 * 8) *reinterpret_cast<float4 *>(Xs + (size_t)(idx >> 3) * XS + (idx & 7) * 4) = v[u];
            }
        }
        __syncthreads();
        const float *wc = wlane + (size_t)kk * 27 * wtap;
#pragma unroll
        for (int m = 0; m < 2; m++) {
            const int q = m ? 7 - wave : wave;
            const int pz = q >> 2, py = (q >> 1) & 1, px = q & 1;
            const float4 *xm = reinterpret_cast<const float4 *>(Xs + (size_t)((m * 5 + (i >> 3)) * 9 + (i & 7)) * XS + h * 16);
            const int ntq = 1 << (pz + py + px);
            auto tap_of = [&](int j, int &t, int &so) {
                const int bz = pz ? (j >> (py + px)) & 1 : 0, by = py ? (j >> px) & 1 : 0, bx = px ? j & 1 : 0;
                const int tz = pz ? (bz ? 2 : 0) : 1, ty = py ? (by ? 2 : 0) : 1, tx = px ? (bx ? 2 : 0) : 1;
                const int dz = (pz && !bz) ? 1 : 0, dyy = (py && !by) ? 1 : 0, dxx = (px && !bx) ? 1 : 0;
                t = (tz * 3 + ty) * 3 + tx;
                so = (dz * 5 + dyy) * 9 + dxx;
            };
            float4 wv[2][4];
            int t0, so0;
            tap_of(0, t0, so0);
#pragma unroll
            for (int e = 0; e < 4; e++) wv[0][e] = *reinterpret_cast<const float4 *>(wc + (size_t)t0 * wtap + e * 4);
            for (int j = 0; j < ntq; j += 2) {
#pragma unroll
                for (int u = 0; u < 2; u++) {
                    if (j + u < ntq) {
                        int t, so, tn, son;
                        tap_of(j + u, t, so);
                        tap_of(j + u + 1 < ntq ? j + u + 1 : j + u, tn, son);
#pragma unroll
                        for (int e = 0; e < 4; e++)
                            wv[(u + 1) & 1][e] = *reinterpret_cast<const float4 *>(wc + (size_t)tn * wtap + e * 4);
                        float4 af[4];
#pragma unroll
                        for (int e = 0; e < 4; e++) af[e] = xm[so * (XS / 4) + e];
#pragma unroll
                        for (int e = 0; e < 4; e++) {
                            acc[m] = __builtin_amdgcn_mfma_f32_32x32x2f32(af[e].x, wv[u][e].x, acc[m], 0, 0, 0);
                            acc[m] = __builtin_amdgcn_mfma_f32_32x32x2f32(af[e].y, wv[u][e].y, acc[m], 0, 0, 0);
                            acc[m] = __builtin_amdgcn_mfma_f32_32x32x2f32(af[e].z, wv[u][e].z, acc[m], 0, 0, 0);
                            acc[m] = __builtin_amdgcn_mfma_f32_32x32x2f32(af[e].w, wv[u][e].w, acc[m], 0, 0, 0);
                        }
                    }
                }
            }
        }
    }
    float *xl = dx + (size_t)(2 * 4 * h) * C + ccol;
#pragma unroll
    for (int m = 0; m < 2; m++) {
        const int q = m ? 7 - wave : wave;
        const int pz = q >> 2, py = (q >> 1) & 1, px = q & 1;
        const int iz = 2 * (oz0 + m) + pz;
#pragma unroll
        for (int r = 0; r < 16; r++) {
            const int iy = 2 * (oy0 + (r >> 2)) + py, ixu = 2 * (ox0 + (r & 3)) + px;
            const size_t uo = ((((size_t)n * g.Dy + iz) * g.Hy + iy) * g.Wy + ixu) * C;
            if (iz < g.Dy && iy < g.Hy && ixu + 8 * h < g.Wy) xl[uo] = tg.acc ? xl[uo] + acc[m][r] : acc[m][r];
        }
    }
}

int dgrad32s(int N, int D, int H, int W, int C, int K, int Do, int Ho, int Wo, const float *dy, const float *wb, float *dx,
             hipStream_t s, int accumulate) {
    if (C % 32 || K % 32 || (((uintptr_t)dy | (uintptr_t)wb) & 15)) return -1;
    if ((long)Do * Ho * Wo * K * 4 >= (1L << 31)) return -1;
    FwdGeom g;
    memset(&g, 0, sizeof(g));
    g.N = N;
    g.Di = Do; g.Hi = Ho; g.Wi = Wo;
    g.Dy = D; g.Hy = H; g.Wy = W;
    g.C1 = K;
    Dg2Tile tg;
    tg.ntd = (Do + 1) / 2; tg.nth = (Ho + 3) / 4; tg.ntw = (Wo + 7) / 8;
    tg.ncb = C / 32;
    tg.C = C;
    tg.acc = accumulate;
    const long nitems = (long)N * tg.ntd * tg.nth * tg.ntw * tg.ncb;
    if (nitems > (1L << 30)) return -1;
    tg.nitems = (int)nitems;
    const unsigned grid = (unsigned)(((nitems + 7) / 8) * 8);
    hipLaunchKernelGGL(k_dgrad32s, dim3(grid), dim3(512), 0, s, g, tg, dy, wb, dx);
    return check_launch("conv dgrad (stride 2, fused parity classes)");
}

static int num_cus();
static int launch_fwd32s(const FwdGeom &g, const float *a1, const float *a2, const float *w, const float *bias, float *y1,
                         float *y2, hipStream_t s) {
    const int K = g.K1 + g.K2;
    Fwd32Tile tg;
    memset(&tg, 0, sizeof(tg));
    int mn[3] = {127, 127, 127}, mx[3] = {-127, -127, -127};
    for (int t = 0; t < g.ntaps; t++)
        for (int a = 0; a < 3; a++) {
            if (g.off[t][a] < mn[a]) mn[a] = g.off[t][a];
            if (g.off[t][a] > mx[a]) mx[a] = g.off[t][a];
        }
    const int T3[3] = {2, 4, 8};
    int E[3];
    for (int a = 0; a < 3; a++) {
        E[a] = (T3[a] - 1) * 2 + (mx[a] - mn[a]) + 1;
        tg.min_off[a] = mn[a];
    }
    tg.EH = E[1]; tg.EW = E[2];
    tg.nslots = E[0] * E[1] * E[2];
    if (tg.nslots > SXR * 64 || g.ntaps != 27) return -1;
    int m = (1 << 16) / tg.EW + 1;
    for (int nn = 0; nn < tg.EH * tg.EW; nn++)
        if (((nn * m) >> 16) != nn / tg.EW) return -1;
    tg.magW = m;
    for (int t = 0; t < g.ntaps; t++)
        tg.toff[t] = ((g.off[t][0] - mn[0]) * tg.EH + (g.off[t][1] - mn[1])) * tg.EW + (g.off[t][2] - mn[2]);
    tg.ntd = (g.Do + 1) / 2;
    tg.nth = (g.Ho + 3) / 4;
    tg.ntw = (g.Wo + 7) / 8;
    tg.nkb = K / 64;
    tg.K = K;
    const long nitems = (long)g.N * tg.ntd * tg.nth * tg.ntw * tg.nkb;
    if (nitems > (1L << 30)) return -1;
    tg.nitems = (int)nitems;
    const size_t lds = (size_t)tg.nslots * 36 * sizeof(float);
    static PerDeviceFlag cfgd;
    if (!cfgd()) {
        if (hipFuncSetAttribute(reinterpret_cast<const void *>(k_fwd32s), hipFuncAttributeMaxDynamicSharedMemorySize,
                                (int)LDS_LIMIT) != hipSuccess) {
            set_error("conv fwd (stride 2): cannot raise the dynamic LDS limit");
            return 1;
        }
        cfgd() = true;
    }
    const unsigned grid = (unsigned)(((nitems + 7) / 8) * 8);
    hipLaunchKernelGGL(k_fwd32s, dim3(grid), dim3(512), lds, s, g, tg, a1, a2, w, bias, y1, y2);
    return check_launch("conv fwd (stride 2, CK=32)");
}

static int num_cus() {
    static int n = 0;
    if (!n) {
        hipDeviceProp_t p;
        int dev = 0;
        if (hipGetDevice(&dev) == hipSuccess && hipGetDeviceProperties(&p, dev) == hipSuccess) n = p.multiProcessorCount;
        if (n <= 0) n = 256;
    }
    return n;
}

static int split_for(const void *ws, size_t ws_bytes, long wgs, int nch, size_t out_elems, int nkb) {
    int S = 1;
    if (ws && wgs < 256 && nch >= 4) {
        long want = 512 / wgs;
        if (want > MAX_SPLIT) want = MAX_SPLIT;
        if (want > nch / 2) want = nch / 2;
        while (want > 1 && (size_t)want * out_elems * sizeof(float) > ws_bytes) want--;
        if (want > 1 && (long)nkb * want <= 65535) S = (int)want;
    }
    return S;
}

static int run_split_reduce(const FwdGeom &g, const float *part, const float *bias, float *y1, float *y2, int S,
                            size_t out_elems, hipStream_t s) {
    long blocks = cdiv((long)out_elems, 256);
    if (blocks > 2048) blocks = 2048;
    hipLaunchKernelGGL(k_split_reduce, dim3(blocks), dim3(256), 0, s, g, part, bias, y1, y2, S);
    return check_launch("conv fwd split reduce");
}
// ... 1900 lines not shown
```

multimodal_mvd_seg_amd/csrc/conv_wino3.hip:

```cpp
#include "common.h"
#include "conv_geom.h"
#include "wino_common.h"

namespace mvd {

typedef float f32x16 __attribute__((ext_vector_type(16)));

__global__ void k_pack_wino3(const float *__restrict__ w, float *__restrict__ uf, float *__restrict__ ub, int K, int C) {
    const long total = (long)64 * C * K;
    const long idx = (long)blockIdx.x * blockDim.x + threadIdx.x;
    if (idx >= total) return;
    const int k = (int)(idx % K);
    const long r = idx / K;
    const int c = (int)(r % C), pos = (int)(r / C);
    pack_wino3_entry(w + ((size_t)k * C + c) * 27, uf, ub, K, C, k, c, pos);
}

int pack_weight_wino3(const float *w, float *uf, float *ub, int K, int C, hipStream_t s) {
    const long total = (long)64 * C * K;
    hipLaunchKernelGGL(k_pack_wino3, dim3(cdiv(total, 256)), dim3(256), 0, s, w, uf, ub, K, C);
    return check_launch("pack_weight_wino3");
}

int wino3_enabled() {
    static int m = -1;
    if (m < 0) m = getenv("MVD_WINO3") ? (atoi(getenv("MVD_WINO3")) != 0) : 1;
    return m;
}

struct Wino3Tile {
    int ntd, nth, ntw, nkb;
    int nth4;
    int nitems;
    int K;
};

constexpr int W3S = 20;
constexpr int W3E = 10;
constexpr int W3P = W3E * W3E;
constexpr int W3IMG = 8 * W3P * W3S;
constexpr int W3XCH = 4 * 4 * 1024;
constexpr int W3ST = (W3IMG > W3XCH ? W3IMG : W3XCH);
constexpr size_t W3LDS = (size_t)(W3ST + 8 * 2 * 64) * sizeof(float);

__global__ __launch_bounds__(512, 1) void k_fwd_wino3(const FwdGeom g, const Wino3Tile tg, const float *__restrict__ a1,
                                                      const float *__restrict__ a2, const float *__restrict__ u,
                                                      const float *__restrict__ bias, float *__restrict__ y1,
                                                      float *__restrict__ y2, float *__restrict__ stats) {
    extern __shared__ __attribute__((aligned(16))) float Xs[];
    const int tid = threadIdx.x, lane = tid & 63;
    const int wave = __builtin_amdgcn_readfirstlane(tid >> 6);
    const int i = lane & 31, h = lane >> 5;
    const int per_xcd = (tg.nitems + 7) >> 3;
    const int item = (int)(blockIdx.x & 7) * per_xcd + (int)(blockIdx.x >> 3);
    if (item >= tg.nitems) return;
    unsigned r_ = (unsigned)item;
    const int kb = __builtin_amdgcn_readfirstlane((int)(r_ % (unsigned)tg.nkb)); r_ /= (unsigned)tg.nkb;
    const int tw_ = __builtin_amdgcn_readfirstlane((int)(r_ % (unsigned)tg.ntw)); r_ /= (unsigned)tg.ntw;
    const int th_ = __builtin_amdgcn_readfirstlane((int)(r_ % (unsigned)tg.nth)); r_ /= (unsigned)tg.nth;
    const int td_ = __builtin_amdgcn_readfirstlane((int)(r_ % (unsigned)tg.ntd));
    const int n = __builtin_amdgcn_readfirstlane((int)(r_ / (unsigned)tg.ntd));

    const int C = g.C1 + g.C2;
    const int nch = C >> 4;
    const int od0 = td_ * 4, oh0 = th_ * 8, ow0 = tw_ * 8;
    const int iz0 = od0 - 1, iy0 = oh0 - 1, ix0 = ow0 - 1;

    const int a = wave & 3, pzh = wave >> 2;
    const int ra = a == 0 ? 0 : (a == 2 ? 2 : 1);
    const int rb = a == 0 ? 2 : (a == 1 ? 2 : (a == 2 ? 1 : 3));
    const float sg = a == 1 ? 1.f : -1.f;
    const v2f sg2 = {sg, sg};
    const int jo = __builtin_popcount(i >> 2) & 1, qr = (i >> 2) & 3, qc = i & 3;
    const int sbase = (jo * 4 + 2 * pzh) * W3P + 2 * qr * W3E + qc;
    const v4f *xa4 = reinterpret_cast<const v4f *>(Xs + (size_t)(sbase + ra * W3E) * W3S + h * 8);
    const v4f *xb4 = reinterpret_cast<const v4f *>(Xs + (size_t)(sbase + rb * W3E) * W3S + h * 8);
    const unsigned uq = 2u * tg.K * 4;
    const unsigned ublk = 4 * uq;
    const unsigned ulane = ((unsigned)(h * tg.K + kb * 32 + i)) << 4;
    const float *uwave = u + (size_t)(16 * pzh + 2 * a) * ublk;

    const bool st_act = tid < 400;
    const int sslot = tid >> 2, squad = tid & 3;
    const int sy = (sslot * 205) >> 11, sx = sslot - sy * W3E;
    const int ih = iy0 + sy, iw = ix0 + sx;
    const bool okyx = st_act && ih >= 0 && ih < g.Hi && iw >= 0 && iw < g.Wi;
    v4f *lds_st = reinterpret_cast<v4f *>(Xs + (size_t)(sy * W3E + (sx >> 1) + 5 * (sx & 1)) * W3S + squad * 4);

    v4f hv[6];
    auto load_halo = [&](int cc) {
        const int c0 = cc * 16;
        const float *src;
        int Cs, cofs;
        if (c0 < g.C1) {
            src = a1; Cs = g.C1; cofs = c0;
        } else {
            src = a2; Cs = g.C2; cofs = c0 - g.C1;
        }
        const unsigned off = (unsigned)((ih * g.Wi + iw) * Cs + cofs + squad * 4) << 2;
#pragma unroll
        for (int z = 0; z < 6; z++) {
            const int id = iz0 + z;
            const float *plane = src + ((size_t)n * g.Di + id) * g.Hi * g.Wi * Cs;
            hv[z] = v4f{0.f, 0.f, 0.f, 0.f};
            if (okyx && id >= 0 && id < g.Di) {
                unsigned o = off;
                asm("" : "+v"(o));
                hv[z] = *reinterpret_cast<const v4f *>(reinterpret_cast<const char *>(plane) + o);
            }
        }
    };

    f32x16 acc[2][4];
#pragma unroll
    for (int p = 0; p < 2; p++)
#pragma unroll
        for (int b = 0; b < 4; b++)
#pragma unroll
            for (int r = 0; r < 16; r++) acc[p][b][r] = 0.f;

    float4 wb[2][4];
#pragma unroll
    for (int b = 0; b < 4; b++)
        wb[0][b] = *reinterpret_cast<const float4 *>(reinterpret_cast<const char *>(uwave + b * uq) + ulane);
    load_halo(0);

    for (int cc = 0; cc < nch; cc++) {
        __syncthreads();
        if (st_act) {
#pragma unroll
            for (int jj = 0; jj < 2; jj++) {
                const v4f d0 = hv[2 * jj], d1 = hv[2 * jj + 1], d2 = hv[2 * jj + 2], d3 = hv[2 * jj + 3];
                lds_st[((jj * 4 + 0) * W3P) * (W3S / 4)] = d0 - d2;
                lds_st[((jj * 4 + 1) * W3P) * (W3S / 4)] = d1 + d2;
                lds_st[((jj * 4 + 2) * W3P) * (W3S / 4)] = d2 - d1;
                lds_st[((jj * 4 + 3) * W3P) * (W3S / 4)] = d1 - d3;
            }
        }
        __syncthreads();
        if (cc + 1 < nch) load_halo(cc + 1);
        const float *uc = uwave + (size_t)cc * 32 * ublk;
        v4f pa[2][4], pb[4];
#pragma unroll
        for (int c = 0; c < 4; c++) {
            pa[0][c] = xa4[w2_coff(c) * (W3S / 4)];
            pb[c] = xb4[w2_coff(c) * (W3S / 4)];
        }
#pragma unroll
        for (int s = 0; s < 4; s++) {
            const int pzl = s >> 1;
            {
                const float *un = s < 3 ? uc + (size_t)((s + 1) >> 1) * 8 * ublk + (size_t)((s + 1) & 1) * ublk
                                        : (cc + 1 < nch ? uc + (size_t)32 * ublk : uc + (size_t)9 * ublk);
                unsigned ul = ulane;
                asm("" : "+v"(ul));
#pragma unroll
                for (int b = 0; b < 4; b++)
                    wb[(s + 1) & 1][b] = *reinterpret_cast<const float4 *>(reinterpret_cast<const char *>(un + b * uq) + ul);
            }
            const int pn = ((s + 1) >> 1) * W3P * (W3S / 4) + ((s + 1) & 1);
            if (s < 3) {
#pragma unroll
                for (int c = 0; c < 4; c++) pa[(s + 1) & 1][c] = xa4[pn + w2_coff(c) * (W3S / 4)];
            }
            __builtin_amdgcn_sched_barrier(0);
            v2f Vl[4], Vh[4];
#pragma unroll
            for (int c = 0; c < 4; c++) {
                Vl[c] = pa[s & 1][c].xy;
                Vh[c] = pa[s & 1][c].zw;
            }
            Vl[1] = wino2_input_transform(sg2, Vl[0], Vl[1], Vl[2], Vl[3], pb[0].xy, pb[1].xy, pb[2].xy, pb[3].xy);
            Vh[1] = wino2_input_transform(sg2, Vh[0], Vh[1], Vh[2], Vh[3], pb[0].zw, pb[1].zw, pb[2].zw, pb[3].zw);
            __builtin_amdgcn_sched_barrier(0);
            if (s < 3) {
#pragma unroll
                for (int c = 0; c < 4; c++) pb[c] = xb4[pn + w2_coff(c) * (W3S / 4)];
            }
            __builtin_amdgcn_sched_barrier(0);
#pragma unroll
            for (int b = 0; b < 4; b++) acc[pzl][b] = __builtin_amdgcn_mfma_f32_32x32x2f32(Vl[b].x, wb[s & 1][b].x, acc[pzl][b], 0, 0, 0);
#pragma unroll
            for (int b = 0; b < 4; b++) acc[pzl][b] = __builtin_amdgcn_mfma_f32_32x32x2f32(Vl[b].y, wb[s & 1][b].y, acc[pzl][b], 0, 0, 0);
#pragma unroll
            for (int b = 0; b < 4; b++) acc[pzl][b] = __builtin_amdgcn_mfma_f32_32x32x2f32(Vh[b].x, wb[s & 1][b].z, acc[pzl][b], 0, 0, 0);
#pragma unroll
            for (int b = 0; b < 4; b++) acc[pzl][b] = __builtin_amdgcn_mfma_f32_32x32x2f32(Vh[b].y, wb[s & 1][b].w, acc[pzl][b], 0, 0, 0);
        }
    }
    const int k = kb * 32 + i;
    const float bv = settled(bias ? bias[k] : 0.f);
    f32x16 t[2][2];
#pragma unroll
    for (int p = 0; p < 2; p++)
#pragma unroll
        for (int r = 0; r < 16; r++) {
            t[p][0][r] = (acc[p][0][r] + acc[p][1][r]) + acc[p][2][r];
            t[p][1][r] = (acc[p][1][r] - acc[p][2][r]) - acc[p][3][r];
        }
    __syncthreads();
    float *xr = Xs + (size_t)a * 4096 + lane;
    if (pzh == 1) {
#pragma unroll
        for (int ox = 0; ox < 2; ox++)
#pragma unroll
            for (int r = 0; r < 16; r++) {
                xr[(0 * 2 + ox) * 1024 + r * 64] = t[0][ox][r];
                xr[(1 * 2 + ox) * 1024 + r * 64] = t[0][ox][r] + t[1][ox][r];
            }
    }
    __syncthreads();
    if (pzh == 0) {
#pragma unroll
        for (int ox = 0; ox < 2; ox++)
#pragma unroll
            for (int r = 0; r < 16; r++) {
                const float m2 = xr[(0 * 2 + ox) * 1024 + r * 64], m23 = xr[(1 * 2 + ox) * 1024 + r * 64];
                xr[(0 * 2 + ox) * 1024 + r * 64] = (t[0][ox][r] + t[1][ox][r]) + m2;
                xr[(1 * 2 + ox) * 1024 + r * 64] = t[1][ox][r] - m23;
            }
    }
    __syncthreads();
    const int oz = wave >> 2, oy = (wave >> 1) & 1, ox = wave & 1;
    const float *xt = Xs + (size_t)(oz * 2 + ox) * 1024 + lane;
    float vals[16];
#pragma unroll
    for (int r = 0; r < 16; r++) {
        const float ta = xt[(size_t)(oy + 0) * 4096 + r * 64], tb = xt[(size_t)(oy + 1) * 4096 + r * 64],
                    tc = xt[(size_t)(oy + 2) * 4096 + r * 64];
        vals[r] = (oy == 0 ? (ta + tb) + tc : (ta - tb) - tc) + bv;
    }
    __builtin_amdgcn_sched_barrier(0);
    float *ylane;
    int Ks;
    if (k < g.K1) {
        ylane = y1 + k; Ks = g.K1;
    } else {
        ylane = y2 + (k - g.K1); Ks = g.K2;
    }
    float ssum[2] = {0.f, 0.f}, ssq[2] = {0.f, 0.f};
#pragma unroll
    for (int r = 0; r < 16; r++) {
        const int m2 = 2 * (r >> 2) + h;
        const int j = __builtin_popcount(m2) & 1, q = m2 & 3;
        const int od = od0 + 2 * j + oz, oh = oh0 + 2 * q + oy, ow = ow0 + 2 * (r & 3) + ox;
        if (od < g.Do && oh < g.Ho && ow < g.Wo) {
            const float val = vals[r];
            ylane[((((size_t)n * g.Dy + od) * g.Hy + oh) * g.Wy + ow) * Ks] = val;
            ssum[(r >> 2) & 1] += val;
            ssq[(r >> 2) & 1] += val * val;
        }
    }
    if (stats != nullptr) {
        float *st = Xs + W3ST;
#pragma unroll
        for (int sb = 0; sb < 2; sb++) {
            ssum[sb] += __shfl_xor(ssum[sb], 32, 64);
            ssq[sb] += __shfl_xor(ssq[sb], 32, 64);
            if (h == 0) {
                st[((wave * 2 + sb) * 32 + i) * 2 + 0] = ssum[sb];
                st[((wave * 2 + sb) * 32 + i) * 2 + 1] = ssq[sb];
            }
        }
        __syncthreads();
        if (wave < 2 && h == 0) {
            const int sb = wave, th4 = 2 * th_ + sb;
            if (th4 < tg.nth4) {
                float sa = 0.f, sq = 0.f;
#pragma unroll
                for (int w = 0; w < 8; w++) {
                    sa += st[((w * 2 + sb) * 32 + i) * 2 + 0];
                    sq += st[((w * 2 + sb) * 32 + i) * 2 + 1];
                }
                const int tile = (td_ * tg.nth4 + th4) * tg.ntw + tw_;
                float *o = stats + (((size_t)n * (tg.ntd * tg.nth4 * tg.ntw) + tile) * tg.K + k) * 2;
                o[0] = sa;
                o[1] = sq;
            }
        }
    }
}

int fwd_wino3(const FwdGeom &g, const float *a1, const float *a2, const float *u, const float *bias, float *y1, float *y2,
              hipStream_t s, float *stats, int *stats_done) {
    if (stats_done) *stats_done = 0;
    const int C = g.C1 + g.C2, K = g.K1 + g.K2;
    if (!u || g.ntaps != 27 || g.T != 27) return -1;
    if (C % 32 || g.C1 % 32 || g.C2 % 32 || K % 32 || g.K1 % 32 || g.K2 % 32) return -1;
    for (int ax = 0; ax < 3; ax++)
        if (g.sa[ax] != 1 || g.so[ax] != 1 || g.oo[ax] != 0) return -1;
    if (g.Dy != g.Do || g.Hy != g.Ho || g.Wy != g.Wo) return -1;
    if (((uintptr_t)a1 | (uintptr_t)a2 | (uintptr_t)u) & 15) return -1;
    if ((long)g.Hi * g.Wi * (C > 0 ? (g.C1 > g.C2 ? g.C1 : g.C2) : 0) * 4 >= (1L << 31)) return -1;
    bool plain = true, mirrored = true;
    for (int t = 0; t < 27; t++) {
        const int oz = g.off[t][0], oy = g.off[t][1], ox = g.off[t][2];
        if (oz < -1 || oz > 1 || oy < -1 || oy > 1 || ox < -1 || ox > 1) return -1;
        const int pos = ((oz + 1) * 3 + (oy + 1)) * 3 + (ox + 1);
        if (g.wt[t] != pos) plain = false;
        if (g.wt[t] != 26 - pos) mirrored = false;
    }
    if (!plain && !mirrored) return -1;
    Wino3Tile tg;
    memset(&tg, 0, sizeof(tg));
    tg.ntd = (g.Do + 3) / 4;
    tg.nth = (g.Ho + 7) / 8;
    tg.ntw = (g.Wo + 7) / 8;
    tg.nth4 = (g.Ho + 3) / 4;
    tg.nkb = K / 32;
    tg.K = K;
    const long nitems = (long)g.N * tg.ntd * tg.nth * tg.ntw * tg.nkb;
    if (nitems > (1L << 30)) return -1;
    tg.nitems = (int)nitems;
    static PerDeviceFlag cfgd;
    if (!cfgd()) {
        if (hipFuncSetAttribute(reinterpret_cast<const void *>(k_fwd_wino3), hipFuncAttributeMaxDynamicSharedMemorySize,
                                (int)W3LDS) != hipSuccess) {
            set_error("conv fwd (winograd 3-D): cannot raise the dynamic LDS limit");
            return 1;
        }
        cfgd() = true;
    }
    const unsigned grid = (unsigned)(((nitems + 7) / 8) * 8);
    float *st = (stats && stats_done && g.K2 == 0) ? stats : nullptr;
    hipLaunchKernelGGL(k_fwd_wino3, dim3(grid), dim3(512), W3LDS, s, g, tg, a1, a2, u, bias, y1, y2, st);
    if (st) *stats_done = 1;
    return check_launch("conv fwd (winograd 3-D)");
}

}
```

multimodal_mvd_seg_amd/csrc/instnorm.hip:

```cpp
#include "common.h"

namespace mvd {

struct NormGeom {
    int C, CG, R, threads, nblk;
    long V, chunk;
};

static NormGeom norm_geom(int N, long V, int C) {
    NormGeom g;
    g.C = C;
    g.V = V;
    int vec = (C % 4 == 0) ? 4 : 1;
    g.CG = C / vec;
    if (g.CG > 256) {
        g.CG = C;
    }
    g.R = 256 / g.CG;
    if (g.R < 1) g.R = 1;
    g.threads = ((g.R * g.CG + 63) / 64) * 64;
    if (g.threads > 1024) g.threads = 1024;
    long want = 2048 / (N > 0 ? N : 1);
    if (want < 1) want = 1;
    long rows_min = (long)g.R * 16;
// ... 538 lines not shown

using namespace mvd;

extern "C" {

int mvd_instnorm_nblk(int N, long V, int C) { return norm_geom(N, V, C).nblk; }

size_t mvd_instnorm_workspace_bytes(int N, long V, int C) {
    NormGeom g = norm_geom(N, V, C);
    return (size_t)N * g.nblk * C * 2 * sizeof(double) + (size_t)N * C * 2 * sizeof(float) + 256;
}

static int in_fwd(const float *x, bool xb, const float *gamma, const float *beta, float *y, bool yb, float *mean,
                  float *rstd, int N, long V, int C, float eps, float slope, void *ws, size_t ws_bytes, void *stream,
                  const float *tile_stats = nullptr, long ntiles = 0) {
    MVD_REQUIRE(x && gamma && beta && y && mean && rstd && ws, "instnorm_fwd: null pointer");
    MVD_REQUIRE(N > 0 && N <= 65535 && V > 0 && C > 0 && C <= 1024, "instnorm_fwd: bad shape N=%d V=%ld C=%d", N, V, C);
    MVD_REQUIRE(ws_bytes >= mvd_instnorm_workspace_bytes(N, V, C), "instnorm_fwd: workspace too small");
    NormGeom g = norm_geom(N, V, C);
    hipStream_t s = as_stream(stream);
    double *partial = reinterpret_cast<double *>(ws);
    size_t sm = (size_t)g.R * C * 2 * sizeof(double);
    MVD_REQUIRE(sm <= 64 * 1024, "instnorm_fwd: C too large for the LDS reduce");
    const bool v4 = (C % 4 == 0) && (g.CG * 4 == C);
    MVD_REQUIRE(v4 || !(xb || yb), "instnorm_fwd: bf16 I/O needs C %% 4 == 0");
    dim3 grid(g.nblk, N);
    if (tile_stats) {
        long nb2 = (ntiles + 63) / 64;
        if (nb2 > g.nblk) nb2 = g.nblk;
        if (nb2 > 64) nb2 = 64;
        const long chunk2 = (ntiles + nb2 - 1) / nb2;
        nb2 = (ntiles + chunk2 - 1) / chunk2;
        const int CW = C < 256 ? C : 256, R2 = 256 / CW;
        hipLaunchKernelGGL(k_in_tiles_reduce, dim3((unsigned)nb2, N), dim3(256), (size_t)R2 * CW * 2 * sizeof(double), s,
                           tile_stats, partial, C, CW, R2, ntiles, chunk2);
        if (check_launch("instnorm statistics from conv tiles")) return 1;
        hipLaunchKernelGGL(k_in_finalize, dim3(C, N), dim3(64), 0, s, partial, mean, rstd, C, (int)nb2, V, eps);
        if (check_launch("instnorm finalize")) return 1;
    } else {
        if (v4 && xb)
            hipLaunchKernelGGL((k_in_stats<4, true>), grid, dim3(g.threads), sm, s, x, partial, C, g.CG, g.R, V, g.chunk);
        else if (v4)
            hipLaunchKernelGGL((k_in_stats<4, false>), grid, dim3(g.threads), sm, s, x, partial, C, g.CG, g.R, V, g.chunk);
        else
            hipLaunchKernelGGL((k_in_stats<1, false>), grid, dim3(g.threads), sm, s, x, partial, C, g.CG, g.R, V, g.chunk);
        if (check_launch("instnorm stats")) return 1;
        float *ss = reinterpret_cast<float *>(partial + (size_t)N * g.nblk * C * 2);
        const bool ssf = v4 && xb && yb;
        hipLaunchKernelGGL(k_in_finalize, dim3(C, N), dim3(64), 0, s, partial, mean, rstd, C, g.nblk, V, eps,
                           ssf ? gamma : nullptr, ssf ? beta : nullptr, ssf ? ss : nullptr, ssf ? ss + (size_t)N * C : nullptr);
        if (check_launch("instnorm finalize")) return 1;
        if (ssf) {
            long nb2 = V / ((long)g.R * 8);
            if (nb2 < 1) nb2 = 1;
            long cap2 = 8192 / N > 0 ? 8192 / N : 1;
            if (nb2 > cap2) nb2 = cap2;
            const long chunk2 = cdiv(V, nb2);
            hipLaunchKernelGGL(k_in_apply_ss16, dim3((unsigned)cdiv(V, chunk2), N), dim3(g.threads), 0, s,
                               reinterpret_cast<const unsigned short *>(x), ss, ss + (size_t)N * C,
                               reinterpret_cast<unsigned short *>(y), C, g.CG, g.R, V, chunk2, slope);
            return check_launch("instnorm apply (scale / shift form)");
        }
    }
    long per_n = V * C / (v4 ? 4 : 1);
    long bx = cdiv(per_n, 256);
    long cap = 4096 / N > 0 ? 4096 / N : 1;
    if (bx > cap) bx = cap;
    if (v4) {
        long nb2 = V / ((long)g.R * 8);
        if (nb2 < 1) nb2 = 1;
        long cap2 = 8192 / N > 0 ? 8192 / N : 1;
        if (nb2 > cap2) nb2 = cap2;
        const long chunk2 = cdiv(V, nb2);
        auto kern = xb ? (yb ? k_in_apply_rows<true, true> : k_in_apply_rows<true, false>)
                       : (yb ? k_in_apply_rows<false, true> : k_in_apply_rows<false, false>);
        hipLaunchKernelGGL(kern, dim3((unsigned)cdiv(V, chunk2), N), dim3(g.threads), 0, s, x, gamma, beta, mean, rstd, y, C,
                           g.CG, g.R, V, chunk2, slope);
    }
    else
        hipLaunchKernelGGL(k_in_apply<1>, dim3(bx, N), dim3(256), 0, s, x, gamma, beta, mean, rstd, y, C, V, slope);
    return check_launch("instnorm apply");
}

static int in_bwd(const float *x, bool xb, const float *dy, bool yb, const float *gamma, const float *beta,
                  const float *mean, const float *rstd, float *dx, float *dgamma, float *dbeta, int N, long V, int C,
                  float slope, void *ws, size_t ws_bytes, void *stream) {
    MVD_REQUIRE(x && dy && gamma && beta && mean && rstd && dx && dgamma && dbeta && ws, "instnorm_bwd: null pointer");
    MVD_REQUIRE(N > 0 && N <= 65535 && V > 0 && C > 0 && C <= 1024, "instnorm_bwd: bad shape");
    MVD_REQUIRE(ws_bytes >= mvd_instnorm_workspace_bytes(N, V, C), "instnorm_bwd: workspace too small");
    NormGeom g = norm_geom(N, V, C);
    hipStream_t s = as_stream(stream);
    double *partial = reinterpret_cast<double *>(ws);
    float *sums = reinterpret_cast<float *>(partial + (size_t)N * g.nblk * C * 2);
    size_t sm = (size_t)g.R * C * 2 * sizeof(double);
    MVD_REQUIRE(sm <= 64 * 1024, "instnorm_bwd: C too large for the LDS reduce");
    const bool v4 = (C % 4 == 0) && (g.CG * 4 == C);
    dim3 grid(g.nblk, N);
    MVD_REQUIRE(v4 || !(xb || yb), "instnorm_bwd: bf16 I/O needs C %% 4 == 0");
    if (v4) {
        auto kern = xb ? (yb ? k_in_bwd_stats<4, true, true> : k_in_bwd_stats<4, true, false>)
                       : (yb ? k_in_bwd_stats<4, false, true> : k_in_bwd_stats<4, false, false>);
        hipLaunchKernelGGL(kern, grid, dim3(g.threads), sm, s, x, dy, gamma, beta, mean, rstd, partial, C, g.CG, g.R, V,
                           g.chunk, slope);
    } else
        hipLaunchKernelGGL((k_in_bwd_stats<1, false, false>), grid, dim3(g.threads), sm, s, x, dy, gamma, beta, mean, rstd,
                           partial, C, g.CG, g.R, V, g.chunk, slope);
    if (check_launch("instnorm bwd stats")) return 1;
    hipLaunchKernelGGL(k_in_bwd_finalize, dim3(C), dim3(64), 0, s, partial, sums, dgamma, dbeta, N, C,
                       g.nblk);
    if (check_launch("instnorm bwd finalize")) return 1;
    long per_n = V * C / (v4 ? 4 : 1);
    long bx = cdiv(per_n, 256);
    long cap = 4096 / N > 0 ? 4096 / N : 1;
    if (bx > cap) bx = cap;
    if (v4) {
        long nb2 = V / ((long)g.R * 8);
        if (nb2 < 1) nb2 = 1;
        long cap2 = 8192 / N > 0 ? 8192 / N : 1;
        if (nb2 > cap2) nb2 = cap2;
        const long chunk2 = cdiv(V, nb2);
        auto kern = xb ? (yb ? k_in_bwd_apply_rows<true, true> : k_in_bwd_apply_rows<true, false>)
                       : (yb ? k_in_bwd_apply_rows<false, true> : k_in_bwd_apply_rows<false, false>);
        hipLaunchKernelGGL(kern, dim3((unsigned)cdiv(V, chunk2), N), dim3(g.threads), 0, s, x, dy, gamma, beta, mean, rstd,
                           sums, dx, C, g.CG, g.R, V, chunk2, slope);
    }
    else
        hipLaunchKernelGGL(k_in_bwd_apply<1>, dim3(bx, N), dim3(256), 0, s, x, dy, gamma, beta, mean, rstd, sums, dx, C,
                           V, slope);
    return check_launch("instnorm bwd apply");
}

int mvd_instnorm_lrelu_fwd(const float *x, const float *gamma, const float *beta, float *y, float *mean, float *rstd,
                           int N, long V, int C, float eps, float slope, void *ws, size_t ws_bytes, void *stream) {
    return in_fwd(x, false, gamma, beta, y, false, mean, rstd, N, V, C, eps, slope, ws, ws_bytes, stream);
}

int mvd_instnorm_lrelu_bwd(const float *x, const float *dy, const float *gamma, const float *beta, const float *mean,
                           const float *rstd, float *dx, float *dgamma, float *dbeta, int N, long V, int C,
                           float slope, void *ws, size_t ws_bytes, void *stream) {
    return in_bwd(x, false, dy, false, gamma, beta, mean, rstd, dx, dgamma, dbeta, N, V, C, slope, ws, ws_bytes, stream);
}

int mvd_instnorm_lrelu_fwd_prestats(const float *x, const float *tile_stats, long ntiles, const float *gamma,
                                    const float *beta, float *y, float *mean, float *rstd, int N, long V, int C, float eps,
                                    float slope, void *ws, size_t ws_bytes, void *stream) {
    MVD_REQUIRE(tile_stats && ntiles > 0, "instnorm_fwd_prestats: tile statistics required");
    return in_fwd(x, false, gamma, beta, y, false, mean, rstd, N, V, C, eps, slope, ws, ws_bytes, stream, tile_stats, ntiles);
}

int mvd_instnorm_finalize_tiles(const float *tile_stats, long ntiles, const float *gamma, const float *beta, float *mean,
                                float *rstd, float *scale, float *shift, int N, long V, int C, float eps, void *stream) {
    MVD_REQUIRE(tile_stats && gamma && beta && mean && rstd && scale && shift, "instnorm_finalize_tiles: null pointer");
    MVD_REQUIRE(ntiles > 0 && N > 0 && N <= 65535 && V > 0 && C > 0 && C <= 65535, "instnorm_finalize_tiles: bad shape");
    hipLaunchKernelGGL(k_in_finalize_tiles, dim3(C, N), dim3(64), 0, as_stream(stream), tile_stats, gamma, beta, mean, rstd,
                       scale, shift, C, ntiles, V, eps);
    return check_launch("instnorm finalize (conv tile statistics)");
}

__global__ void k_in_scale_shift(const float *__restrict__ gamma, const float *__restrict__ beta, const float *__restrict__ mean,
                                 const float *__restrict__ rstd, float *__restrict__ scale, float *__restrict__ shift, int N,
                                 int C) {
    const int i = blockIdx.x * blockDim.x + threadIdx.x;
    if (i >= N * C) return;
    const float sc = gamma[i % C] * rstd[i];
    scale[i] = sc;
    shift[i] = fmaf(-mean[i], sc, beta[i % C]);
}

int mvd_instnorm_stats_bf16(const void *x, int x_is_bf16, const float *gamma, const float *beta, float *mean, float *rstd,
                            float *scale, float *shift, int N, long V, int C, float eps, void *ws, size_t ws_bytes,
                            void *stream) {
    MVD_REQUIRE(x && gamma && beta && mean && rstd && scale && shift && ws, "instnorm_stats: null pointer");
    MVD_REQUIRE(N > 0 && N <= 65535 && V > 0 && C > 0 && C % 4 == 0 && C <= 1024, "instnorm_stats: bad shape (C %% 4 == 0)");
    MVD_REQUIRE(ws_bytes >= mvd_instnorm_workspace_bytes(N, V, C), "instnorm_stats: workspace too small");
    NormGeom g = norm_geom(N, V, C);
    MVD_REQUIRE(g.CG * 4 == C, "instnorm_stats: C too wide");
    hipStream_t s = as_stream(stream);
    double *partial = reinterpret_cast<double *>(ws);
    const size_t sm = (size_t)g.R * C * 2 * sizeof(double);
    MVD_REQUIRE(sm <= 64 * 1024, "instnorm_stats: C too large for the LDS reduce");
    const float *xf = reinterpret_cast<const float *>(x);
    if (x_is_bf16)
        hipLaunchKernelGGL((k_in_stats<4, true>), dim3(g.nblk, N), dim3(g.threads), sm, s, xf, partial, C, g.CG, g.R, V, g.chunk);
    else
        hipLaunchKernelGGL((k_in_stats<4, false>), dim3(g.nblk, N), dim3(g.threads), sm, s, xf, partial, C, g.CG, g.R, V, g.chunk);
    if (check_launch("instnorm stats")) return 1;
    hipLaunchKernelGGL(k_in_finalize, dim3(C, N), dim3(64), 0, s, partial, mean, rstd, C, g.nblk, V, eps, gamma, beta, scale, shift);
    return check_launch("instnorm finalize");
}

int mvd_instnorm_stats_from_tiles(const float *tile_stats, long ntiles, float *mean, float *rstd, int N, long V, int C, float eps,
                                  void *ws, size_t ws_bytes, void *stream) {
    MVD_REQUIRE(tile_stats && ntiles > 0 && mean && rstd && ws, "instnorm_stats_from_tiles: bad arguments");
    MVD_REQUIRE(N > 0 && N <= 65535 && V > 0 && C > 0 && C <= 1024, "instnorm_stats_from_tiles: bad shape");
    MVD_REQUIRE(ws_bytes >= mvd_instnorm_workspace_bytes(N, V, C), "instnorm_stats_from_tiles: workspace too small");
    NormGeom g = norm_geom(N, V, C);
    hipStream_t s = as_stream(stream);
    double *partial = reinterpret_cast<double *>(ws);
    long nb2 = (ntiles + 63) / 64;
    if (nb2 > g.nblk) nb2 = g.nblk;
    if (nb2 > 64) nb2 = 64;
    const long chunk2 = (ntiles + nb2 - 1) / nb2;
    nb2 = (ntiles + chunk2 - 1) / chunk2;
    const int CW = C < 256 ? C : 256, R2 = 256 / CW;
    hipLaunchKernelGGL(k_in_tiles_reduce, dim3((unsigned)nb2, N), dim3(256), (size_t)R2 * CW * 2 * sizeof(double), s, tile_stats,
                       partial, C, CW, R2, ntiles, chunk2);
    if (check_launch("instnorm statistics from conv tiles")) return 1;
    hipLaunchKernelGGL(k_in_finalize, dim3(C, N), dim3(64), 0, s, partial, mean, rstd, C, (int)nb2, V, eps);
    return check_launch("instnorm finalize");
}

int mvd_instnorm_lrelu_apply_bf16(const uint16_t *x, const float *scale, const float *shift, uint16_t *y, int N, long V,
                                  int C, float slope, void *stream) {
    MVD_REQUIRE(x && scale && shift && y, "instnorm_apply_bf16: null pointer");
    MVD_REQUIRE(N > 0 && N <= 65535 && V > 0 && C > 0 && C % 4 == 0 && C <= 1024, "instnorm_apply_bf16: bad shape (C %% 4 == 0)");
    NormGeom g = norm_geom(N, V, C);
    MVD_REQUIRE(g.CG * 4 == C, "instnorm_apply_bf16: C too wide");
    long nb2 = V / ((long)g.R * 8);
    if (nb2 < 1) nb2 = 1;
    long cap2 = 8192 / N > 0 ? 8192 / N : 1;
    if (nb2 > cap2) nb2 = cap2;
    const long chunk2 = cdiv(V, nb2);
    hipLaunchKernelGGL(k_in_apply_ss16, dim3((unsigned)cdiv(V, chunk2), N), dim3(g.threads), 0, as_stream(stream), x, scale,
                       shift, y, C, g.CG, g.R, V, chunk2, slope);
// ... 18 lines not shown
```

multimodal_mvd_seg_amd/ops.py:

```python
import ctypes
import os
import typing
import weakref

import numpy as np
import torch
from torch.autograd import Function
from torch.autograd.function import once_differentiable

from . import _lib
from ._lib import call, i3, query

CL3D = torch.channels_last_3d


def _stream():
    return ctypes.c_void_p(torch.cuda.current_stream().cuda_stream)


def _p(t):
    return ctypes.c_void_p(t.data_ptr()) if t is not None else None


def _require_cuda(*ts):
# ... 330 lines not shown
    wb_ = PA(*[ptr(e.wb) for _, e, _w in jobs])
    uf_ = PA(*[ptr(e.uf) for _, e, _w in jobs])
    ub_ = PA(*[ptr(e.ub) for _, e, _w in jobs])
    vf_ = PA(*[ptr(e.vf) for _, e, _w in jobs])
    vb_ = PA(*[ptr(e.vb) for _, e, _w in jobs])
    K_ = IA(*[e.K for _, e, _w in jobs])
    C_ = IA(*[e.C for _, e, _w in jobs])
    T_ = IA(*[e.T for _, e, _w in jobs])
    tr_ = IA(*[1 if e.transposed else 0 for _, e, _w in jobs])
    cast = lambda a: ctypes.cast(a, ctypes.c_void_p)
    call("mvd_pack_weights_batch3", n, cast(w_), cast(wf_), cast(wb_), cast(uf_), cast(ub_), cast(vf_), cast(vb_), cast(K_),
         cast(C_), cast(T_), cast(tr_), _stream())
    for d, e, w in jobs:
        e.stamp = _pack_stamp(d, w)
        e.gen += 1


def pack_weight_bf16(weight, transposed):
    w = weight.detach()
    if not w.is_contiguous():
        w = w.contiguous()
    if transposed:
        C, K = w.shape[:2]
    else:
        K, C = w.shape[:2]
    T = w[0, 0].numel()
    wf = torch.empty((T * C * K,), dtype=BF16, device=w.device)
    wb = torch.empty((T * C * K,), dtype=BF16, device=w.device)
    call("mvd_pack_weight_bf16", _p(w), _p(wf), _p(wb), K, C, T, 1 if transposed else 0, _stream())
    return wf, wb


def _packed_bf16(weight, transposed):
    w = weight.detach()
    if not w.is_contiguous():
        return pack_weight_bf16(weight, transposed)
    e = getattr(weight, "_mvd_pack16", None)
    key = (_pack_stamp(w, weight), transposed, w.device)
    if e is None or e.key != key:
        if e is None:
            if len(_PACK16_LIVE) >= 4096:
                _PACK16_LIVE[:] = [r for r in _PACK16_LIVE if r() is not None]
            _PACK16_LIVE.append(weakref.ref(weight))
        if e is not None and e.inplace and e.key[1:] == key[1:]:
            e = _pack16_rewrite(weight, e, _pack16_shape(w, transposed=transposed))
        else:
            e = _Pack16(key, *pack_weight_bf16(weight, transposed))
        weight._mvd_pack16 = e
    return e.wf, e.wb


def _out_dim(i, k, s):
    return (i + 2 * ((k - 1) // 2) - k) // s + 1


class _GradShare:
    __slots__ = ("buf",)

    def __init__(self):
        self.buf = None


def share_grad(t):
    if t.requires_grad:
        t._mvd_gshare = _GradShare()
    return t


def _share_of(t):
    return getattr(t, "_mvd_gshare", None)


def _publish(share, dx):
    if share is not None:
        share.buf = dx
    return dx


def _joinable(share, shape, dtype):
    b = share.buf if share is not None else None
    return b if (b is not None and tuple(b.shape) == tuple(shape) and b.dtype == dtype and _is_cl3d(b)) else None


class LaunchTimer:

    def __init__(self, key):
        self.key, self.pairs, self.on = tuple(key), [], False

    def mean_ms(self):
        return sum(a.elapsed_time(b) for a, b in self.pairs) / len(self.pairs) if self.pairs else None


LAUNCH_TIMER = None


BF16_CONV_STATS = [os.environ.get("MVD_BF16_CONV_STATS", "1") != "0"]


def conv3d_fwd_bf16(x1, C1, x2, C2, wf, bias, y, N, D, H, W, K, ks, stride, ws, in_scale=None, in_shift=None, slope=0.01):
    nt = query("mvd_conv3d_fwd_bf16_stats_tiles", N, D, H, W, C1, C2, K, i3(ks), i3(stride)) \
        if (BF16_CONV_STATS[0] or in_scale is not None) else 0
    if nt <= 0 and in_scale is None:
        call("mvd_conv3d_fwd_bf16", _p(x1), C1, _p(x2), C2, _p(wf), _p(bias), _p(y), N, D, H, W, K, i3(ks), i3(stride),
             _p(ws), ws.numel(), _stream())
        return
    stats = torch.empty((N, nt, K, 2), dtype=torch.float32, device=y.device) if (nt > 0 and BF16_CONV_STATS[0]) else None
    got = ctypes.c_int(0)
    call("mvd_conv3d_fwd_bf16_fused", _p(x1), C1, _p(x2), C2, _p(wf), _p(bias), _p(y), N, D, H, W, K, i3(ks), i3(stride),
         _p(in_scale), _p(in_shift), float(slope), _p(stats), ctypes.byref(got), _p(ws), ws.numel(), _stream())
    if stats is not None and got.value > 0:
        y._mvd_tile_stats16 = (stats, int(got.value))


class Conv3dFn(Function):

    @staticmethod
    def forward(ctx, x1, x2, weight, bias, stride):
        _require_cuda(x1, x2, weight, bias)
        ctx.share1, ctx.share2 = _share_of(x1), (_share_of(x2) if x2 is not None else None)
        x1 = to_ndhwc(x1)
        x2 = to_ndhwc(x2) if x2 is not None else None
        K, C = weight.shape[:2]
        ks = tuple(weight.shape[2:])
        N, C1, D, H, W = x1.shape
        C2 = x2.shape[1] if x2 is not None else 0
        if C1 + C2 != C:
            raise RuntimeError(f"conv3d: weight expects {C} input channels, got {C1}+{C2}")
        if x2 is not None and tuple(x2.shape[2:]) != (D, H, W):
            raise RuntimeError("conv3d: the two concatenated inputs differ in spatial size")
        bf = _is_bf16(x1)
        if x2 is not None and _is_bf16(x2) != bf:
            raise RuntimeError("conv3d: the two concatenated inputs differ in dtype")
        od = [_out_dim(i, k, s) for i, k, s in zip((D, H, W), ks, stride)]
        y = empty_cl3d((N, K, *od), x1.device, x1.dtype)
        ws = _Workspace.get(query("mvd_conv_fwd_workspace_bytes", N, od[0] * od[1] * od[2], K), x1.device)
        ub = None
        tm = LAUNCH_TIMER
        timed = tm is not None and tm.on and tm.key == (bf, N, C1, C2, K, D, H, W, tuple(ks), tuple(stride))
        if timed:
            ev0 = torch.cuda.Event(enable_timing=True)
            ev0.record()
        if bf:
            wf, wb = _packed_bf16(weight, False)
            conv3d_fwd_bf16(x1, C1, x2, C2, wf, bias, y, N, D, H, W, K, ks, stride, ws)
        else:
            wino = query("mvd_conv_wino_applicable", N, D, H, W, C1, C2, K, i3(ks), i3(stride)) if len(ks) == 3 else 0
            wino3 = query("mvd_conv_wino3_applicable", N, D, H, W, C1, C2, K, i3(ks), i3(stride)) if wino else 0
            wino2 = wino & ~wino3
            pk = _packed(weight, False, bool(wino2 & 1), bool(wino2 & 2), bool(wino3 & 1), bool(wino3 & 2))
            wf, wb = pk.wf, pk.wb
            uf = pk.vf if wino3 & 1 else (pk.uf if wino2 & 1 else None)
            ub = pk.vb if wino3 & 2 else (pk.ub if wino2 & 2 else None)
            sfx3 = "3" if wino3 & 1 else ""
            ctx.ub3 = bool(wino3 & 2)
            if uf is not None:
                ntiles = query("mvd_conv_stats_tiles", od[0], od[1], od[2])
                stats = torch.empty((N, ntiles, K, 2), dtype=torch.float32, device=x1.device)
                done = ctypes.c_int(0)
                call("mvd_conv3d_fwd_wino" + sfx3 + "_stats", _p(x1), C1, _p(x2), C2, _p(wf), _p(uf), _p(bias), _p(y),
                     _p(stats), ctypes.byref(done), N, D, H, W, K, i3(ks), i3(stride), _p(ws), ws.numel(), _stream())
                if done.value:
                    y._mvd_tile_stats = (stats, ntiles)
            else:
                call("mvd_conv3d_fwd_wino", _p(x1), C1, _p(x2), C2, _p(wf), _p(uf), _p(bias), _p(y), N, D, H, W, K, i3(ks),
                     i3(stride), _p(ws), ws.numel(), _stream())
        if timed:
            ev1 = torch.cuda.Event(enable_timing=True)
            ev1.record()
            tm.pairs.append((ev0, ev1))
        ctx.bf = bf
        ctx.params = (weight, bias)
        ctx.pack = None if bf else (pk, pk.gen)
        ctx.pack16_gen = _pack16_guard(weight) if bf else None
        ctx.save_for_backward(x1, x2, wb, ub)
        ctx.geom = (N, C1, C2, D, H, W, K, ks, tuple(stride), tuple(od), bias is not None)
        return y

    @staticmethod
    @once_differentiable
    def backward(ctx, dy):
        x1, x2, wb, ub = ctx.saved_tensors
        _check_pack_generation(ctx.pack, "conv3d backward")
        _check_pack16_generation(ctx.pack16_gen, "conv3d backward")
        N, C1, C2, D, H, W, K, ks, stride, od, has_bias = ctx.geom
        dy = to_ndhwc(dy)
        dev = dy.device
        sfx = "_bf16" if ctx.bf else ""
        dx1 = dx2 = dw = db = None
        need1, need2 = ctx.needs_input_grad[0], (x2 is not None and ctx.needs_input_grad[1])
        joined = None
        if need1 and x2 is None and len(ks) == 3:
            joined = _joinable(ctx.share1, (N, C1, D, H, W), dy.dtype)
            if joined is not None and not query("mvd_conv3d_dgrad_acc_ok", int(ctx.bf), N, D, H, W, C1, K, i3(ks), i3(stride)):
                joined = None
        if joined is not None:
            if ctx.bf:
                ws = _Workspace.get(query("mvd_conv_fwd_workspace_bytes", N, D * H * W, C1), dev)
                call("mvd_conv3d_dgrad_bf16_acc", _p(dy), _p(wb), _p(joined), C1, N, D, H, W, K, i3(ks), i3(stride), _p(ws),
                     ws.numel(), _stream())
            else:
                call("mvd_conv3d_dgrad_acc", _p(dy), _p(wb), _p(joined), C1, N, D, H, W, K, i3(ks), i3(stride), _stream())
            ctx.share1.buf = None
            need1 = False
        elif need1 or need2:
            dx1 = empty_cl3d((N, C1, D, H, W), dev, dy.dtype)
            dx2 = empty_cl3d((N, C2, D, H, W), dev, dy.dtype) if x2 is not None else None
            ws = _Workspace.get(query("mvd_conv_fwd_workspace_bytes", N, D * H * W, C1 + C2), dev)
            if ctx.bf:
                call("mvd_conv3d_dgrad_bf16", _p(dy), _p(wb), _p(dx1), C1, _p(dx2), C2, N, D, H, W, K, i3(ks), i3(stride),
                     _p(ws), ws.numel(), _stream())
            else:
                call("mvd_conv3d_dgrad_wino3" if ctx.ub3 else "mvd_conv3d_dgrad_wino", _p(dy), _p(wb), _p(ub), _p(dx1), C1,
                     _p(dx2), C2, N, D, H, W, K, i3(ks), i3(stride), _p(ws), ws.numel(), _stream())
            if need1:
                _publish(ctx.share1, dx1)
            if need2:
                _publish(ctx.share2, dx2)
        if ctx.needs_input_grad[2]:
            T = ks[0] * ks[1] * ks[2]
            weight, bias = ctx.params
            sink_w, sink_b = _take_grad(weight), (_take_grad(bias) if has_bias else None)
            dw = sink_w if sink_w is not None else torch.empty((K, C1 + C2, *ks), dtype=torch.float32, device=dev)
            db = (sink_b if sink_b is not None else torch.empty((K,), dtype=torch.float32, device=dev)) if has_bias else None
            nb = query("mvd_conv3d_wgrad_workspace_bytes", C1 + C2, K, T, N, *od)
            ws = _Workspace.get(nb, dev)
            call("mvd_conv3d_wgrad" + sfx, _p(x1), C1, _p(x2), C2, _p(dy), _p(dw), _p(db), N, D, H, W, K, i3(ks), i3(stride),
                 _p(ws), ws.numel(), _stream())
            if sink_w is not None:
                dw = None
                _grad_done(weight)
            if sink_b is not None:
                db = None
                _grad_done(bias)
        return (dx1 if need1 else None), (dx2 if need2 else None), dw, db, None


def _padded_pack_bf16(weight, cpad):
    w = weight.detach()

    def fresh(src):
        K, T = src.shape[0], src[0, 0].numel()
        wf = torch.empty((T * cpad * K,), dtype=BF16, device=src.device)
        wb = torch.empty((T * cpad * K,), dtype=BF16, device=src.device)
        _pack16_launch([(src, wf, wb) + _pack16_shape(src, cpad=cpad)], src.device)
        return wf, wb

    if not w.is_contiguous() or w.dtype != torch.float32:
        return fresh(w.float().contiguous())
    e = getattr(weight, "_mvd_pack16pad", None)
    key = (_pack_stamp(w, weight), cpad, w.device)
    if e is None or e.key != key:
        if e is None:
            if len(_PACK16PAD_LIVE) >= 4096:
                _PACK16PAD_LIVE[:] = [r for r in _PACK16PAD_LIVE if r() is not None]
            _PACK16PAD_LIVE.append(weakref.ref(weight))
        if e is not None and e.inplace and e.key[1:] == key[1:]:
            e = _pack16_rewrite(weight, e, _pack16_shape(w, cpad=cpad))
        else:
            e = _Pack16(key, *fresh(w))
        weight._mvd_pack16pad = e
    return e.wf, e.wb


class NarrowInputConv3dBf16Fn(Function):
    CPAD = 32

    @staticmethod
    def forward(ctx, x, weight, bias):
        _require_cuda(x, weight, bias)
        if x.dtype != torch.float32:
            raise RuntimeError("narrow-input bf16 conv: the network input must be fp32")
        if ctx.needs_input_grad[0]:
            raise RuntimeError("narrow-input bf16 conv: the gradient with respect to the network input is not on the path "
                               "(detach the input, or run the layer in fp32)")
        K, C = weight.shape[:2]
        if tuple(weight.shape[2:]) != (3, 3, 3) or K % 32 != 0 or C > 8 or x.shape[1] != C:
            raise RuntimeError("narrow-input bf16 conv: needs a 3x3x3 conv with <= 8 input and a multiple of 32 output channels")
        N, _, D, H, W = x.shape
        cl = _is_cl3d(x)
        if not cl and not x.is_contiguous():
            x = x.contiguous()
        cp = NarrowInputConv3dBf16Fn.CPAD
        xp = empty_cl3d((N, cp, D, H, W), x.device, BF16)
        call("mvd_pad_channels_bf16", _p(x), _p(xp), N, C, cp, D * H * W, 1 if cl else 0, _stream())
        wf, _wb = _padded_pack_bf16(weight, cp)
        y = empty_cl3d((N, K, D, H, W), x.device, BF16)
        ws = _Workspace.get(query("mvd_conv_fwd_workspace_bytes", N, D * H * W, K), x.device)
        conv3d_fwd_bf16(xp, cp, None, 0, wf, bias, y, N, D, H, W, K, (3, 3, 3), (1, 1, 1), ws)
        ctx.save_for_backward(xp)
        ctx.params = (weight, bias)
        ctx.geom = (N, C, D, H, W, K)
        return y

    @staticmethod
    @once_differentiable
    def backward(ctx, dy):
# ... 46 lines not shown
        ws = _Workspace.get(query("mvd_conv_fwd_workspace_bytes", N, D * H * W, K), x.device)
        ctx.bf = bf
        ctx.params = (weight, bias)
        ctx.pack = None if bf else (pk, pk.gen)
        ctx.pack16_gen = _pack16_guard(weight) if bf else None
        call("mvd_convT3d_fwd_bf16" if bf else "mvd_convT3d_fwd", _p(x), _p(wf), _p(bias), _p(y), N, D, H, W, C, K, i3(stride), _p(ws), ws.numel(),
             _stream())
        ctx.save_for_backward(x, wb)
        ctx.geom = (N, C, K, D, H, W, tuple(stride), bias is not None)
        return y

    @staticmethod
    @once_differentiable
    def backward(ctx, dy):
        x, wb = ctx.saved_tensors
        _check_pack_generation(ctx.pack, "convT3d backward")
        _check_pack16_generation(ctx.pack16_gen, "convT3d backward")
        N, C, K, D, H, W, stride, has_bias = ctx.geom
        dy = to_ndhwc(dy)
        dev = dy.device
        dx = dw = db = None
        sfx = "_bf16" if ctx.bf else ""
        if ctx.needs_input_grad[0]:
            dx = empty_cl3d((N, C, D, H, W), dev, dy.dtype)
            ws = _Workspace.get(query("mvd_conv_fwd_workspace_bytes", N, D * H * W, C), dev)
            call("mvd_convT3d_dgrad" + sfx, _p(dy), _p(wb), _p(dx), N, D, H, W, C, K, i3(stride), _p(ws), ws.numel(),
                 _stream())
            _publish(ctx.share, dx)
        if ctx.needs_input_grad[1]:
            T = stride[0] * stride[1] * stride[2]
            weight, bias = ctx.params
            sink_w, sink_b = _take_grad(weight), (_take_grad(bias) if has_bias else None)
            dw = sink_w if sink_w is not None else torch.empty((C, K, *stride), dtype=torch.float32, device=dev)
            db = (sink_b if sink_b is not None else torch.empty((K,), dtype=torch.float32, device=dev)) if has_bias else None
            nb = query("mvd_convT3d_wgrad_workspace_bytes", C, K, T, N, D, H, W)
            ws = _Workspace.get(nb, dev)
            call("mvd_convT3d_wgrad" + sfx, _p(x), _p(dy), _p(dw), _p(db), N, D, H, W, C, K, i3(stride), _p(ws), ws.numel(),
                 _stream())
            if sink_w is not None:
                dw = None
                _grad_done(weight)
            if sink_b is not None:
                db = None
                _grad_done(bias)
        return dx, dw, db, None


class InstanceNormLeakyReLUFn(Function):

    @staticmethod
    def forward(ctx, x, gamma, beta, eps, slope, out_bf16=False):
        _require_cuda(x, gamma, beta)
        x = to_ndhwc(x)
        N, C = x.shape[:2]
        V = x[0, 0].numel()
        xb = _is_bf16(x)
        yb = bool(out_bf16) or xb
        y = empty_cl3d(x.shape, x.device, BF16 if yb else torch.float32)
        mean = torch.empty((N, C), dtype=torch.float32, device=x.device)
        rstd = torch.empty((N, C), dtype=torch.float32, device=x.device)
        nb = query("mvd_instnorm_workspace_bytes", N, V, C)
        ws = _Workspace.get(nb, x.device)
        g, b = gamma.detach().contiguous(), beta.detach().contiguous()
        pre = getattr(x, '_mvd_tile_stats', None)
        pre16 = getattr(x, '_mvd_tile_stats16', None) if xb else None
        if pre16 is not None and pre16[0].shape[0] == N and pre16[0].shape[2] == C and C % 4 == 0:
            scale, shift = torch.empty_like(mean), torch.empty_like(mean)
            call("mvd_instnorm_finalize_tiles", _p(pre16[0]), pre16[1], _p(g), _p(b), _p(mean), _p(rstd), _p(scale),
                 _p(shift), N, V, C, float(eps), _stream())
            call("mvd_instnorm_lrelu_apply_bf16", _p(x), _p(scale), _p(shift), _p(y), N, V, C, float(slope), _stream())
        elif yb:
            call("mvd_instnorm_lrelu_fwd_bf16", _p(x), int(xb), _p(g), _p(b), _p(y), _p(mean), _p(rstd), N, V, C,
                 float(eps), float(slope), _p(ws), ws.numel(), _stream())
        elif pre is not None and pre[0].shape[0] == N and pre[0].shape[2] == C:
            call("mvd_instnorm_lrelu_fwd_prestats", _p(x), _p(pre[0]), pre[1], _p(g), _p(b), _p(y), _p(mean), _p(rstd), N, V,
                 C, float(eps), float(slope), _p(ws), ws.numel(), _stream())
        else:
            call("mvd_instnorm_lrelu_fwd", _p(x), _p(g), _p(b), _p(y), _p(mean), _p(rstd), N, V, C, float(eps),
                 float(slope), _p(ws), ws.numel(), _stream())
        ctx.save_for_backward(x, g, b, mean, rstd)
        ctx.slope = float(slope)
        ctx.yb = yb
        ctx.params = (gamma, beta)
        return y

    @staticmethod
    @once_differentiable
    def backward(ctx, dy):
        x, g, b, mean, rstd = ctx.saved_tensors
        dy = to_ndhwc(dy)
        N, C = x.shape[:2]
        V = x[0, 0].numel()
        dx = empty_cl3d(x.shape, x.device, x.dtype)
        gamma, beta = ctx.params
        sink_g = _take_grad(gamma) if ctx.needs_input_grad[1] else None
        sink_b = _take_grad(beta) if ctx.needs_input_grad[2] else None
        dg = sink_g if sink_g is not None else torch.empty((C,), dtype=torch.float32, device=x.device)
        db = sink_b if sink_b is not None else torch.empty((C,), dtype=torch.float32, device=x.device)
        nb = query("mvd_instnorm_workspace_bytes", N, V, C)
        ws = _Workspace.get(nb, x.device)
        if ctx.yb:
            call("mvd_instnorm_lrelu_bwd_bf16", _p(x), int(_is_bf16(x)), _p(dy), _p(g), _p(b), _p(mean), _p(rstd), _p(dx),
                 _p(dg), _p(db), N, V, C, ctx.slope, _p(ws), ws.numel(), _stream())
        else:
            call("mvd_instnorm_lrelu_bwd", _p(x), _p(dy), _p(g), _p(b), _p(mean), _p(rstd), _p(dx), _p(dg), _p(db), N, V,
                 C, ctx.slope, _p(ws), ws.numel(), _stream())
        if sink_g is not None:
            dg = None
            _grad_done(gamma)
        if sink_b is not None:
            db = None
            _grad_done(beta)
        return dx, dg, db, None, None, None


WGRAD_PROLOGUE = os.environ.get("MVD_WGRAD_PROLOGUE", "1") != "0"


class NormActConv3dFn(Function):

    @staticmethod
    def forward(ctx, y0, gamma, beta, eps, slope, weight, bias):
        _require_cuda(y0, gamma, beta, weight, bias)
        pre = getattr(y0, '_mvd_tile_stats16', None)
        if not (_is_bf16(y0) and _is_cl3d(y0)):
            raise RuntimeError("NormActConv3dFn: needs the raw bf16 NDHWC conv output")
        N, C, D, H, W = y0.shape
        K = weight.shape[0]
        V = D * H * W
        if tuple(weight.shape[1:]) != (C, 3, 3, 3):
            raise RuntimeError("NormActConv3dFn: 3x3x3 conv over the normalised tensor's channels")
        g, b = gamma.detach().contiguous(), beta.detach().contiguous()
        mean = torch.empty((N, C), dtype=torch.float32, device=y0.device)
        rstd, scale, shift = torch.empty_like(mean), torch.empty_like(mean), torch.empty_like(mean)
        tm = LAUNCH_TIMER
        timed = tm is not None and tm.on and tm.key == (True, N, C, 0, K, D, H, W, (3, 3, 3), (1, 1, 1))
        if timed:
            ev0 = torch.cuda.Event(enable_timing=True)
            ev0.record()
        if pre is not None and pre[0].shape[0] == N and pre[0].shape[2] == C:
            call("mvd_instnorm_finalize_tiles", _p(pre[0]), pre[1], _p(g), _p(b), _p(mean), _p(rstd), _p(scale), _p(shift), N,
                 V, C, float(eps), _stream())
        else:
            ws = _Workspace.get(query("mvd_instnorm_workspace_bytes", N, V, C), y0.device)
            call("mvd_instnorm_stats_bf16", _p(y0), 1, _p(g), _p(b), _p(mean), _p(rstd), _p(scale), _p(shift), N, V, C,
                 float(eps), _p(ws), ws.numel(), _stream())
        wf, wb = _packed_bf16(weight, False)
        y1 = empty_cl3d((N, K, D, H, W), y0.device, BF16)
        ws = _Workspace.get(query("mvd_conv_fwd_workspace_bytes", N, V, K), y0.device)
        conv3d_fwd_bf16(y0, C, None, 0, wf, bias, y1, N, D, H, W, K, (3, 3, 3), (1, 1, 1), ws, scale, shift, slope)
        if timed:
            ev1 = torch.cuda.Event(enable_timing=True)
            ev1.record()
            tm.pairs.append((ev0, ev1))
        ctx.save_for_backward(y0, g, b, mean, rstd, scale, shift, wb)
        ctx.params = (gamma, beta, weight, bias)
        ctx.slope = float(slope)
        ctx.pack16_gen = _pack16_guard(weight)
        return y1

    @staticmethod
    @once_differentiable
    def backward(ctx, dy1):
        y0, g, b, mean, rstd, scale, shift, wb = ctx.saved_tensors
        _check_pack16_generation(ctx.pack16_gen, "norm+act+conv3d backward")
        gamma, beta, weight, bias = ctx.params
        N, C, D, H, W = y0.shape
        K = weight.shape[0]
        V = D * H * W
        dev = y0.device
        dy1 = to_ndhwc(dy1)
        ks, st = i3((3, 3, 3)), i3((1, 1, 1))
        dy0 = dg = db_ = dw = db = None
        if ctx.needs_input_grad[0] or ctx.needs_input_grad[1] or ctx.needs_input_grad[2]:
            da0 = empty_cl3d((N, C, D, H, W), dev, BF16)
            ws = _Workspace.get(query("mvd_conv_fwd_workspace_bytes", N, V, C), dev)
            call("mvd_conv3d_dgrad_bf16", _p(dy1), _p(wb), _p(da0), C, None, 0, N, D, H, W, K, ks, st, _p(ws), ws.numel(),
                 _stream())
            dy0 = empty_cl3d(y0.shape, dev, BF16)
            sink_g, sink_b = _take_grad(gamma), _take_grad(beta)
            dg = sink_g if sink_g is not None else torch.empty((C,), dtype=torch.float32, device=dev)
            db_ = sink_b if sink_b is not None else torch.empty((C,), dtype=torch.float32, device=dev)
            ws = _Workspace.get(query("mvd_instnorm_workspace_bytes", N, V, C), dev)
            call("mvd_instnorm_lrelu_bwd_bf16", _p(y0), 1, _p(da0), _p(g), _p(b), _p(mean), _p(rstd), _p(dy0), _p(dg), _p(db_),
                 N, V, C, ctx.slope, _p(ws), ws.numel(), _stream())
            if sink_g is not None:
                dg = None
                _grad_done(gamma)
            if sink_b is not None:
# ... 863 lines not shown
```

Baseline: 60.49 samples/s.

## Fuse instance-norm backward reductions into conv dgrad epilogues

The conv dgrad kernels (the Winograd-3 stride-1 path and the accumulating stride-2 path) now compute per-tile sums of dz and dz*xhat for the following InstanceNorm+LeakyReLU backward while they write dx. The norm backward then reduces those tile sums instead of re-reading x and dy in a separate stats pass. This is meant to remove a full-tensor read pass per norm layer. In exchange it adds tagging plumbing between the autograd functions and extra epilogue work and shared-memory reductions in the dgrad kernels. Selection is limited to certain voxel ranges and channel counts.

```diff
diff --git a/include/mvdseg_hip.h b/include/mvdseg_hip.h
--- a/include/mvdseg_hip.h
+++ b/include/mvdseg_hip.h
@@ -101,6 +101,22 @@
                          const int ksize[3], const int stride[3], void *stream);
 int mvd_conv3d_dgrad_bf16_acc(const uint16_t *dy, const uint16_t *wb, uint16_t *dx1, int C1, int N, int D, int H, int W, int K,
                               const int ksize[3], const int stride[3], void *ws, size_t ws_bytes, void *stream);
+int mvd_conv3d_dgrad_wino3_bwdstats(const float *dy, const float *wb, const float *vb, float *dx1, int C1, float *dx2, int C2,
+                                    int N, int D, int H, int W, int K, const int ksize[3], const int stride[3],
+                                    const float *xn, const float *mean, const float *rstd, const float *gamma,
+                                    const float *beta, float slope, float *tiles, int *done, void *ws, size_t ws_bytes,
+                                    void *stream);
+long mvd_conv3d_dgrad_acc_sum_tiles(int D, int H, int W);
+int mvd_conv3d_dgrad_acc_bwdstats(const float *dy, const float *wb, float *dx1, int C1, int N, int D, int H, int W, int K,
+                                  const int ksize[3], const int stride[3], const float *xn, const float *mean,
+                                  const float *rstd, const float *gamma, const float *beta, float slope, float *tiles,
+                                  void *stream);
+int mvd_instnorm_lrelu_bwd_prestats(const float *x, const float *dy, const float *tile_sums, long ntiles, const float *gamma,
+                                    const float *beta, const float *mean, const float *rstd, float *dx, float *dgamma,
+                                    float *dbeta, int N, long V, int C, float slope, void *ws, size_t ws_bytes, void *stream);
+long mvd_in_bwd_prestats_launches(void);
+int mvd_set_in_bwd_prestats_voxels(int kind, long lo, long hi);
+int mvd_in_bwd_prestats_select(int kind, int N, int D, int H, int W, int C);
 int mvd_set_bf16_zmarch_kernel(int which);
 int mvd_set_bf16_wgrad_kernel(int which);
 int mvd_conv3d_wgrad_bf16_prologue_ok(int N, int D, int H, int W, int C1, int C2, int K, const int ksize[3], const int stride[3]);
diff --git a/multimodal_mvd_seg_amd/_lib.py b/multimodal_mvd_seg_amd/_lib.py
--- a/multimodal_mvd_seg_amd/_lib.py
+++ b/multimodal_mvd_seg_amd/_lib.py
@@ -50,6 +50,16 @@
                                            _I3, _I3, _P, c_size_t, _P]),
     "mvd_conv3d_dgrad_wino3": (c_int, [_P, _P, _P, _P, c_int, _P, c_int, c_int, c_int, c_int, c_int, c_int, _I3, _I3, _P,
                                        c_size_t, _P]),
+    "mvd_conv3d_dgrad_wino3_bwdstats": (c_int, [_P, _P, _P, _P, c_int, _P, c_int, c_int, c_int, c_int, c_int, c_int, _I3, _I3,
+                                                _P, _P, _P, _P, _P, c_float, _P, _P, _P, c_size_t, _P]),
+    "mvd_conv3d_dgrad_acc_sum_tiles": (c_long, [c_int, c_int, c_int]),
+    "mvd_conv3d_dgrad_acc_bwdstats": (c_int, [_P, _P, _P, c_int, c_int, c_int, c_int, c_int, c_int, _I3, _I3, _P, _P, _P, _P,
+                                              _P, c_float, _P, _P]),
+    "mvd_instnorm_lrelu_bwd_prestats": (c_int, [_P, _P, _P, c_long, _P, _P, _P, _P, _P, _P, _P, c_int, c_long, c_int, c_float,
+                                                _P, c_size_t, _P]),
+    "mvd_in_bwd_prestats_launches": (c_long, []),
+    "mvd_set_in_bwd_prestats_voxels": (c_int, [c_int, c_long, c_long]),
+    "mvd_in_bwd_prestats_select": (c_int, [c_int, c_int, c_int, c_int, c_int, c_int]),
     "mvd_set_wgrad_wino3_min_items": (c_int, [c_long]),
     "mvd_conv_wgrad_wino3_applicable": (c_int, [c_int, c_int, c_int, c_int, c_int, c_int, c_int, _I3, _I3]),
     "mvd_wgrad_wino3_launches": (c_long, []),
diff --git a/multimodal_mvd_seg_amd/csrc/conv.hip b/multimodal_mvd_seg_amd/csrc/conv.hip
--- a/multimodal_mvd_seg_amd/csrc/conv.hip
+++ b/multimodal_mvd_seg_amd/csrc/conv.hip
@@ -291,12 +291,12 @@
 
 static int run_fwd(const FwdGeom &g, const float *a1, const float *a2, const float *w, const float *bias, float *y1,
                    float *y2, void *ws, size_t ws_bytes, hipStream_t s, const float *u = nullptr, float *stats = nullptr,
-                   int *stats_done = nullptr, bool u3d = false) {
+                   int *stats_done = nullptr, bool u3d = false, const InBwdSums *bw = nullptr) {
     if (stats_done) *stats_done = 0;
     if (u3d) {
         if (g_engine_mode == 0 && u && !g_wino_off && wino3_enabled() &&
             wino3_items(g.Do, g.Ho, g.Wo, g.K1 + g.K2) >= g_wino3_min_items) {
-            int r = fwd_wino3(g, a1, a2, u, bias, y1, y2, s, stats, stats_done);
+            int r = fwd_wino3(g, a1, a2, u, bias, y1, y2, s, stats, stats_done, bw);
             if (r >= 0) return r;
             if (stats_done) *stats_done = 0;
         }
@@ -498,7 +498,8 @@
 
 static int conv3d_dgrad_impl(const float *dy, const float *wb, const float *ub, float *dx1, int C1, float *dx2, int C2,
                              int N, int D, int H, int W, int K, const int ksize[3], const int stride[3], void *ws,
-                             size_t ws_bytes, void *stream, bool u3d = false);
+                             size_t ws_bytes, void *stream, bool u3d = false, const InBwdSums *bw = nullptr,
+                             int *bw_done = nullptr);
 
 int mvd_conv3d_dgrad(const float *dy, const float *wb, float *dx1, int C1, float *dx2, int C2, int N, int D, int H, int W,
                      int K, const int ksize[3], const int stride[3], void *ws, size_t ws_bytes, void *stream) {
@@ -517,9 +518,23 @@
     return conv3d_dgrad_impl(dy, wb, vb, dx1, C1, dx2, C2, N, D, H, W, K, ksize, stride, ws, ws_bytes, stream, true);
 }
 
+int mvd_conv3d_dgrad_wino3_bwdstats(const float *dy, const float *wb, const float *vb, float *dx1, int C1, float *dx2, int C2,
+                                    int N, int D, int H, int W, int K, const int ksize[3], const int stride[3],
+                                    const float *xn, const float *mean, const float *rstd, const float *gamma,
+                                    const float *beta, float slope, float *tiles, int *done, void *ws, size_t ws_bytes,
+                                    void *stream) {
+    MVD_REQUIRE(dx2 == nullptr && C2 == 0, "conv3d_dgrad_wino3_bwdstats: single-input convs only (dx2 must be null)");
+    MVD_REQUIRE(xn && mean && rstd && gamma && beta && tiles && done, "conv3d_dgrad_wino3_bwdstats: null pointer");
+    MVD_REQUIRE(ksize && stride && stride[0] == 1 && stride[1] == 1 && stride[2] == 1, "conv3d_dgrad_wino3_bwdstats: stride 1 only");
+    *done = 0;
+    InBwdSums bw;
+    bw.xn = xn; bw.mean = mean; bw.rstd = rstd; bw.gamma = gamma; bw.beta = beta; bw.slope = slope; bw.tiles = tiles;
+    return conv3d_dgrad_impl(dy, wb, vb, dx1, C1, nullptr, 0, N, D, H, W, K, ksize, stride, ws, ws_bytes, stream, true, &bw, done);
+}
+
 static int conv3d_dgrad_impl(const float *dy, const float *wb, const float *ub, float *dx1, int C1, float *dx2, int C2,
                              int N, int D, int H, int W, int K, const int ksize[3], const int stride[3], void *ws,
-                             size_t ws_bytes, void *stream, bool u3d) {
+                             size_t ws_bytes, void *stream, bool u3d, const InBwdSums *bw, int *bw_done) {
     MVD_REQUIRE(dy && wb && dx1 && C1 > 0 && C2 >= 0 && (C2 == 0 || dx2), "conv3d_dgrad: null pointer / bad channels");
     MVD_REQUIRE(N > 0 && D > 0 && H > 0 && W > 0 && K > 0, "conv3d_dgrad: bad shape");
     if (check_ks(ksize, stride, "conv3d_dgrad")) return 2;
@@ -577,8 +592,8 @@
                 g.ntaps = nt;
                 g.T = ksize[0] * ksize[1] * ksize[2];
                 if (nt == 0) continue;
-                int r = run_fwd(g, dy, nullptr, wb, nullptr, dx1, dx2, ws, ws_bytes, as_stream(stream), ub, nullptr, nullptr,
-                                u3d);
+                int r = run_fwd(g, dy, nullptr, wb, nullptr, dx1, dx2, ws, ws_bytes, as_stream(stream), ub, nullptr, bw_done,
+                                u3d, bw);
                 if (r) return r;
             }
     return 0;
@@ -969,6 +984,41 @@
     return r;
 }
 
+long mvd_conv3d_dgrad_acc_sum_tiles(int D, int H, int W) { return (D > 0 && H > 0 && W > 0) ? dgrad32s_sum_tiles(D, H, W) : 0; }
+
+int mvd_conv3d_dgrad_acc_bwdstats(const float *dy, const float *wb, float *dx1, int C1, int N, int D, int H, int W, int K,
+                                  const int ksize[3], const int stride[3], const float *xn, const float *mean,
+                                  const float *rstd, const float *gamma, const float *beta, float slope, float *tiles,
+                                  void *stream) {
+    MVD_REQUIRE(dy && wb && dx1 && xn && mean && rstd && gamma && beta && tiles, "conv3d_dgrad_acc_bwdstats: null pointer");
+    MVD_REQUIRE(mvd_conv3d_dgrad_acc_ok(0, N, D, H, W, C1, K, ksize, stride), "conv3d_dgrad_acc_bwdstats: no accumulating kernel for "
+                "this shape (ask mvd_conv3d_dgrad_acc_ok first)");
+    InBwdSums bw;
+    bw.xn = xn; bw.mean = mean; bw.rstd = rstd; bw.gamma = gamma; bw.beta = beta; bw.slope = slope; bw.tiles = tiles;
+    int r = dgrad32s(N, D, H, W, C1, K, out_dim(D, 3, 2), out_dim(H, 3, 2), out_dim(W, 3, 2), dy, wb, dx1, as_stream(stream), 1, &bw);
+    if (r < 0) {
+        set_error("conv3d_dgrad_acc_bwdstats: the fused stride-2 kernel refused the shape");
+        return 3;
+    }
+    return r;
+}
+
+static const long kInBwdVoxDefault[2][2] = {{0, 32L * 32 * 32}, {1, 0}};
+static long g_in_bwd_vox[2][2] = {{kInBwdVoxDefault[0][0], kInBwdVoxDefault[0][1]}, {kInBwdVoxDefault[1][0], kInBwdVoxDefault[1][1]}};
+
+int mvd_set_in_bwd_prestats_voxels(int kind, long lo, long hi) {
+    MVD_REQUIRE(kind == 0 || kind == 1, "set_in_bwd_prestats_voxels: kind must be 0 or 1");
+    g_in_bwd_vox[kind][0] = lo < 0 ? kInBwdVoxDefault[kind][0] : lo;
+    g_in_bwd_vox[kind][1] = hi < 0 ? kInBwdVoxDefault[kind][1] : hi;
+    return 0;
+}
+
+int mvd_in_bwd_prestats_select(int kind, int N, int D, int H, int W, int C) {
+    if ((kind != 0 && kind != 1) || N <= 0 || D <= 0 || H <= 0 || W <= 0 || C <= 0 || C % 32 || C > 1024) return 0;
+    const long v = (long)D * H * W;
+    return (v >= g_in_bwd_vox[kind][0] && v <= g_in_bwd_vox[kind][1]) ? 1 : 0;
+}
+
 int mvd_convT3d_fwd_bf16(const uint16_t *x, const uint16_t *wf, const float *bias, uint16_t *y, int N, int D, int H, int W, int C, int K,
                     const int stride[3], void *ws, size_t ws_bytes, void *stream) {
     MVD_REQUIRE(x && wf && y && N > 0 && D > 0 && H > 0 && W > 0 && C > 0 && K > 0, "convT3d_fwd_bf16: bad arguments");
diff --git a/multimodal_mvd_seg_amd/csrc/conv_geom.h b/multimodal_mvd_seg_amd/csrc/conv_geom.h
--- a/multimodal_mvd_seg_amd/csrc/conv_geom.h
+++ b/multimodal_mvd_seg_amd/csrc/conv_geom.h
@@ -1,5 +1,6 @@
 #pragma once
 #include <stdint.h>
+#include <type_traits>
 
 namespace mvd {
 
@@ -56,12 +57,19 @@
 int fwd_wino(const FwdGeom &g, const float *a1, const float *a2, const float *u, const float *bias, float *y1, float *y2,
              hipStream_t s, float *stats = nullptr, int *stats_done = nullptr);
 int pack_weight_wino(const float *w, float *uf, float *ub, int K, int C, hipStream_t s);
+struct InBwdSums {
+    const float *xn = nullptr, *mean = nullptr, *rstd = nullptr, *gamma = nullptr, *beta = nullptr;
+    float slope = 0.f;
+    float *tiles = nullptr;
+};
+struct NoBwdSums {};
 int fwd_wino3(const FwdGeom &g, const float *a1, const float *a2, const float *u, const float *bias, float *y1, float *y2,
-              hipStream_t s, float *stats = nullptr, int *stats_done = nullptr);
+              hipStream_t s, float *stats = nullptr, int *stats_done = nullptr, const InBwdSums *bw = nullptr);
 int pack_weight_wino3(const float *w, float *uf, float *ub, int K, int C, hipStream_t s);
 int wino3_enabled();
 int dgrad32s(int N, int D, int H, int W, int C, int K, int Do, int Ho, int Wo, const float *dy, const float *wb, float *dx,
-             hipStream_t s, int accumulate = 0);
+             hipStream_t s, int accumulate = 0, const InBwdSums *bw = nullptr);
+long dgrad32s_sum_tiles(int D, int H, int W);
 int dgrad16s(int N, int D, int H, int W, int C, int K, int Do, int Ho, int Wo, const unsigned short *dy, const unsigned short *wb,
              unsigned short *dx, hipStream_t s, int accumulate = 0);
 int launch_fwd16ys(const FwdGeom &g, const unsigned short *a1, const unsigned short *a2, const unsigned short *w, const float *bias,
diff --git a/multimodal_mvd_seg_amd/csrc/conv_mfma.hip b/multimodal_mvd_seg_amd/csrc/conv_mfma.hip
--- a/multimodal_mvd_seg_amd/csrc/conv_mfma.hip
+++ b/multimodal_mvd_seg_amd/csrc/conv_mfma.hip
@@ -625,8 +625,10 @@
     int ntd, nth, ntw, ncb, nitems, C;
     int acc;
 };
+template <bool BWS>
 __global__ __launch_bounds__(512, 2) void k_dgrad32s(const FwdGeom g, const Dg2Tile tg, const float *__restrict__ dy,
-                                                     const float *__restrict__ wb, float *__restrict__ dx) {
+                                                     const float *__restrict__ wb, float *__restrict__ dx,
+                                                     const std::conditional_t<BWS, InBwdSums, NoBwdSums> bw) {
     __shared__ __attribute__((aligned(16))) float Xs[135 * 36];
     constexpr int XS = 36;
     const int tid = threadIdx.x, lane = tid & 63;
@@ -723,23 +725,93 @@
         }
     }
     float *xl = dx + (size_t)(2 * 4 * h) * C + ccol;
-#pragma unroll
-    for (int m = 0; m < 2; m++) {
-        const int q = m ? 7 - wave : wave;
-        const int pz = q >> 2, py = (q >> 1) & 1, px = q & 1;
-        const int iz = 2 * (oz0 + m) + pz;
-#pragma unroll
-        for (int r = 0; r < 16; r++) {
-            const int iy = 2 * (oy0 + (r >> 2)) + py, ixu = 2 * (ox0 + (r & 3)) + px;
-            const size_t uo = ((((size_t)n * g.Dy + iz) * g.Hy + iy) * g.Wy + ixu) * C;
-            if (iz < g.Dy && iy < g.Hy && ixu + 8 * h < g.Wy) xl[uo] = tg.acc ? xl[uo] + acc[m][r] : acc[m][r];
-        }
-    }
+    if constexpr (BWS) {
+        const float *xnl = bw.xn + (size_t)(2 * 4 * h) * C + ccol;
+        const float mu = bw.mean[(size_t)n * C + ccol], rs = bw.rstd[(size_t)n * C + ccol];
+        const float ga = bw.gamma[ccol], be = bw.beta[ccol];
+        float sa[2] = {0.f, 0.f}, sq[2] = {0.f, 0.f};
+#pragma unroll
+        for (int m = 0; m < 2; m++) {
+            const int q = m ? 7 - wave : wave;
+            const int pz = q >> 2, py = (q >> 1) & 1, px = q & 1;
+            const int iz = 2 * (oz0 + m) + pz;
+            float xo[16], xq[16];
+#pragma unroll
+            for (int r = 0; r < 16; r++) {
+                const int iy = 2 * (oy0 + (r >> 2)) + py, ixu = 2 * (ox0 + (r & 3)) + px;
+                const size_t uo = ((((size_t)n * g.Dy + iz) * g.Hy + iy) * g.Wy + ixu) * C;
+                xo[r] = xq[r] = 0.f;
+                if (iz < g.Dy && iy < g.Hy && ixu + 8 * h < g.Wy) {
+                    xo[r] = xl[uo];
+                    xq[r] = xnl[uo];
+                }
+            }
+#pragma unroll
+            for (int r = 0; r < 16; r++) {
+                const int iy = 2 * (oy0 + (r >> 2)) + py, ixu = 2 * (ox0 + (r & 3)) + px;
+                const size_t uo = ((((size_t)n * g.Dy + iz) * g.Hy + iy) * g.Wy + ixu) * C;
+                if (iz < g.Dy && iy < g.Hy && ixu + 8 * h < g.Wy) {
+                    const float val = xo[r] + acc[m][r];
+                    xl[uo] = val;
+                    const float xh = (xq[r] - mu) * rs;
+                    const float z = fmaf(xh, ga, be);
+                    const float dz = z > 0.f ? val : val * bw.slope;
+                    sa[m] += dz;
+                    sq[m] += dz * xh;
+                }
+            }
+        }
+        __syncthreads();
+#pragma unroll
+        for (int m = 0; m < 2; m++) {
+            sa[m] += __shfl_xor(sa[m], 32, 64);
+            sq[m] += __shfl_xor(sq[m], 32, 64);
+            if (h == 0) {
+                Xs[((wave * 2 + m) * 32 + i) * 2 + 0] = sa[m];
+                Xs[((wave * 2 + m) * 32 + i) * 2 + 1] = sq[m];
+            }
+        }
+        __syncthreads();
+        if (wave < 4 && h == 0) {
+            const int zl = wave, m = zl >> 1, pz = zl & 1;
+            const int w0 = 4 * (m ? 1 - pz : pz);
+            float ta = 0.f, tq = 0.f;
+#pragma unroll
+            for (int w = 0; w < 4; w++) {
+                ta += Xs[(((w0 + w) * 2 + m) * 32 + i) * 2 + 0];
+                tq += Xs[(((w0 + w) * 2 + m) * 32 + i) * 2 + 1];
+            }
+            const size_t ntiles = (size_t)4 * tg.ntd * tg.nth * tg.ntw;
+            const size_t tile = ((size_t)(4 * td_ + zl) * tg.nth + th_) * tg.ntw + tw_;
+            float *o = bw.tiles + ((n * ntiles + tile) * C + ccol) * 2;
+            o[0] = ta;
+            o[1] = tq;
+        }
+    } else {
+#pragma unroll
+        for (int m = 0; m < 2; m++) {
+            const int q = m ? 7 - wave : wave;
+            const int pz = q >> 2, py = (q >> 1) & 1, px = q & 1;
+            const int iz = 2 * (oz0 + m) + pz;
+#pragma unroll
+            for (int r = 0; r < 16; r++) {
+                const int iy = 2 * (oy0 + (r >> 2)) + py, ixu = 2 * (ox0 + (r & 3)) + px;
+                const size_t uo = ((((size_t)n * g.Dy + iz) * g.Hy + iy) * g.Wy + ixu) * C;
+                if (iz < g.Dy && iy < g.Hy && ixu + 8 * h < g.Wy) xl[uo] = tg.acc ? xl[uo] + acc[m][r] : acc[m][r];
+            }
+        }
+    }
+}
+
+long dgrad32s_sum_tiles(int D, int H, int W) {
+    const int Do = (D - 1) / 2 + 1, Ho = (H - 1) / 2 + 1, Wo = (W - 1) / 2 + 1;
+    return 4L * ((Do + 1) / 2) * ((Ho + 3) / 4) * ((Wo + 7) / 8);
 }
 
 int dgrad32s(int N, int D, int H, int W, int C, int K, int Do, int Ho, int Wo, const float *dy, const float *wb, float *dx,
-             hipStream_t s, int accumulate) {
+             hipStream_t s, int accumulate, const InBwdSums *bw) {
     if (C % 32 || K % 32 || (((uintptr_t)dy | (uintptr_t)wb) & 15)) return -1;
+    if (bw && !(accumulate && bw->xn && bw->mean && bw->rstd && bw->gamma && bw->beta && bw->tiles)) return -1;
     if ((long)Do * Ho * Wo * K * 4 >= (1L << 31)) return -1;
     FwdGeom g;
     memset(&g, 0, sizeof(g));
@@ -756,7 +828,10 @@
     if (nitems > (1L << 30)) return -1;
     tg.nitems = (int)nitems;
     const unsigned grid = (unsigned)(((nitems + 7) / 8) * 8);
-    hipLaunchKernelGGL(k_dgrad32s, dim3(grid), dim3(512), 0, s, g, tg, dy, wb, dx);
+    if (bw)
+        hipLaunchKernelGGL(k_dgrad32s<true>, dim3(grid), dim3(512), 0, s, g, tg, dy, wb, dx, *bw);
+    else
+        hipLaunchKernelGGL(k_dgrad32s<false>, dim3(grid), dim3(512), 0, s, g, tg, dy, wb, dx, NoBwdSums{});
     return check_launch("conv dgrad (stride 2, fused parity classes)");
 }
 
diff --git a/multimodal_mvd_seg_amd/csrc/conv_wino3.hip b/multimodal_mvd_seg_amd/csrc/conv_wino3.hip
--- a/multimodal_mvd_seg_amd/csrc/conv_wino3.hip
+++ b/multimodal_mvd_seg_amd/csrc/conv_wino3.hip
@@ -43,10 +43,12 @@
 constexpr int W3ST = (W3IMG > W3XCH ? W3IMG : W3XCH);
 constexpr size_t W3LDS = (size_t)(W3ST + 8 * 2 * 64) * sizeof(float);
 
+template <bool BWD>
 __global__ __launch_bounds__(512, 1) void k_fwd_wino3(const FwdGeom g, const Wino3Tile tg, const float *__restrict__ a1,
                                                       const float *__restrict__ a2, const float *__restrict__ u,
                                                       const float *__restrict__ bias, float *__restrict__ y1,
-                                                      float *__restrict__ y2, float *__restrict__ stats) {
+                                                      float *__restrict__ y2, float *__restrict__ stats,
+                                                      const std::conditional_t<BWD, InBwdSums, NoBwdSums> bw) {
     extern __shared__ __attribute__((aligned(16))) float Xs[];
     const int tid = threadIdx.x, lane = tid & 63;
     const int wave = __builtin_amdgcn_readfirstlane(tid >> 6);
@@ -190,6 +192,27 @@
     }
     const int k = kb * 32 + i;
     const float bv = settled(bias ? bias[k] : 0.f);
+    const int oz = wave >> 2, oy = (wave >> 1) & 1, ox = wave & 1;
+    auto out_voxel = [&](int r, size_t &ov) {
+        const int m2 = 2 * (r >> 2) + h;
+        const int j = __builtin_popcount(m2) & 1, q = m2 & 3;
+        const int od = od0 + 2 * j + oz, oh = oh0 + 2 * q + oy, ow = ow0 + 2 * (r & 3) + ox;
+        ov = (((size_t)n * g.Dy + od) * g.Hy + oh) * g.Wy + ow;
+        return od < g.Do && oh < g.Ho && ow < g.Wo;
+    };
+    float xv[BWD ? 16 : 1], mu = 0.f, rs = 0.f, ga = 0.f, be = 0.f;
+    if constexpr (BWD) {
+#pragma unroll
+        for (int r = 0; r < 16; r++) {
+            size_t ov;
+            xv[r] = 0.f;
+            if (out_voxel(r, ov)) xv[r] = bw.xn[ov * g.K1 + k];
+        }
+        mu = bw.mean[(size_t)n * g.K1 + k];
+        rs = bw.rstd[(size_t)n * g.K1 + k];
+        ga = bw.gamma[k];
+        be = bw.beta[k];
+    }
     f32x16 t[2][2];
 #pragma unroll
     for (int p = 0; p < 2; p++)
@@ -221,7 +244,6 @@
             }
     }
     __syncthreads();
-    const int oz = wave >> 2, oy = (wave >> 1) & 1, ox = wave & 1;
     const float *xt = Xs + (size_t)(oz * 2 + ox) * 1024 + lane;
     float vals[16];
 #pragma unroll
@@ -241,17 +263,23 @@
     float ssum[2] = {0.f, 0.f}, ssq[2] = {0.f, 0.f};
 #pragma unroll
     for (int r = 0; r < 16; r++) {
-        const int m2 = 2 * (r >> 2) + h;
-        const int j = __builtin_popcount(m2) & 1, q = m2 & 3;
-        const int od = od0 + 2 * j + oz, oh = oh0 + 2 * q + oy, ow = ow0 + 2 * (r & 3) + ox;
-        if (od < g.Do && oh < g.Ho && ow < g.Wo) {
+        size_t ov;
+        if (out_voxel(r, ov)) {
             const float val = vals[r];
-            ylane[((((size_t)n * g.Dy + od) * g.Hy + oh) * g.Wy + ow) * Ks] = val;
-            ssum[(r >> 2) & 1] += val;
-            ssq[(r >> 2) & 1] += val * val;
-        }
-    }
-    if (stats != nullptr) {
+            ylane[ov * Ks] = val;
+            if constexpr (BWD) {
+                const float xh = (xv[r] - mu) * rs;
+                const float z = fmaf(xh, ga, be);
+                const float dz = z > 0.f ? val : val * bw.slope;
+                ssum[(r >> 2) & 1] += dz;
+                ssq[(r >> 2) & 1] += dz * xh;
+            } else {
+                ssum[(r >> 2) & 1] += val;
+                ssq[(r >> 2) & 1] += val * val;
+            }
+        }
+    }
+    if (BWD || stats != nullptr) {
         float *st = Xs + W3ST;
 #pragma unroll
         for (int sb = 0; sb < 2; sb++) {
@@ -282,7 +310,7 @@
 }
 
 int fwd_wino3(const FwdGeom &g, const float *a1, const float *a2, const float *u, const float *bias, float *y1, float *y2,
-              hipStream_t s, float *stats, int *stats_done) {
+              hipStream_t s, float *stats, int *stats_done, const InBwdSums *bw) {
     if (stats_done) *stats_done = 0;
     const int C = g.C1 + g.C2, K = g.K1 + g.K2;
     if (!u || g.ntaps != 27 || g.T != 27) return -1;
@@ -314,7 +342,9 @@
     tg.nitems = (int)nitems;
     static PerDeviceFlag cfgd;
     if (!cfgd()) {
-        if (hipFuncSetAttribute(reinterpret_cast<const void *>(k_fwd_wino3), hipFuncAttributeMaxDynamicSharedMemorySize,
+        if (hipFuncSetAttribute(reinterpret_cast<const void *>(k_fwd_wino3<false>), hipFuncAttributeMaxDynamicSharedMemorySize,
+                                (int)W3LDS) != hipSuccess ||
+            hipFuncSetAttribute(reinterpret_cast<const void *>(k_fwd_wino3<true>), hipFuncAttributeMaxDynamicSharedMemorySize,
                                 (int)W3LDS) != hipSuccess) {
             set_error("conv fwd (winograd 3-D): cannot raise the dynamic LDS limit");
             return 1;
@@ -322,8 +352,13 @@
         cfgd() = true;
     }
     const unsigned grid = (unsigned)(((nitems + 7) / 8) * 8);
+    if (bw && stats_done && g.K2 == 0 && bw->xn && bw->mean && bw->rstd && bw->gamma && bw->beta && bw->tiles) {
+        hipLaunchKernelGGL(k_fwd_wino3<true>, dim3(grid), dim3(512), W3LDS, s, g, tg, a1, a2, u, bias, y1, y2, bw->tiles, *bw);
+        *stats_done = 1;
+        return check_launch("conv dgrad (winograd 3-D, InstanceNorm backward sums)");
+    }
     float *st = (stats && stats_done && g.K2 == 0) ? stats : nullptr;
-    hipLaunchKernelGGL(k_fwd_wino3, dim3(grid), dim3(512), W3LDS, s, g, tg, a1, a2, u, bias, y1, y2, st);
+    hipLaunchKernelGGL(k_fwd_wino3<false>, dim3(grid), dim3(512), W3LDS, s, g, tg, a1, a2, u, bias, y1, y2, st, NoBwdSums{});
     if (st) *stats_done = 1;
     return check_launch("conv fwd (winograd 3-D)");
 }
diff --git a/multimodal_mvd_seg_amd/csrc/instnorm.hip b/multimodal_mvd_seg_amd/csrc/instnorm.hip
--- a/multimodal_mvd_seg_amd/csrc/instnorm.hip
+++ b/multimodal_mvd_seg_amd/csrc/instnorm.hip
@@ -644,9 +644,11 @@
     return check_launch("instnorm apply");
 }
 
+static long g_in_bwd_prestats_launches = 0;
+
 static int in_bwd(const float *x, bool xb, const float *dy, bool yb, const float *gamma, const float *beta,
                   const float *mean, const float *rstd, float *dx, float *dgamma, float *dbeta, int N, long V, int C,
-                  float slope, void *ws, size_t ws_bytes, void *stream) {
+                  float slope, void *ws, size_t ws_bytes, void *stream, const float *tile_sums = nullptr, long ntiles = 0) {
     MVD_REQUIRE(x && dy && gamma && beta && mean && rstd && dx && dgamma && dbeta && ws, "instnorm_bwd: null pointer");
     MVD_REQUIRE(N > 0 && N <= 65535 && V > 0 && C > 0 && C <= 1024, "instnorm_bwd: bad shape");
     MVD_REQUIRE(ws_bytes >= mvd_instnorm_workspace_bytes(N, V, C), "instnorm_bwd: workspace too small");
@@ -659,7 +661,20 @@
     const bool v4 = (C % 4 == 0) && (g.CG * 4 == C);
     dim3 grid(g.nblk, N);
     MVD_REQUIRE(v4 || !(xb || yb), "instnorm_bwd: bf16 I/O needs C %% 4 == 0");
-    if (v4) {
+    int nblk = g.nblk;
+    if (tile_sums) {
+        long nb2 = (ntiles + 63) / 64;
+        if (nb2 > g.nblk) nb2 = g.nblk;
+        if (nb2 > 64) nb2 = 64;
+        const long chunk2 = (ntiles + nb2 - 1) / nb2;
+        nb2 = (ntiles + chunk2 - 1) / chunk2;
+        const int CW = C < 256 ? C : 256, R2 = 256 / CW;
+        hipLaunchKernelGGL(k_in_tiles_reduce, dim3((unsigned)nb2, N), dim3(256), (size_t)R2 * CW * 2 * sizeof(double), s,
+                           tile_sums, partial, C, CW, R2, ntiles, chunk2);
+        if (check_launch("instnorm bwd sums from conv tiles")) return 1;
+        nblk = (int)nb2;
+        g_in_bwd_prestats_launches++;
+    } else if (v4) {
         auto kern = xb ? (yb ? k_in_bwd_stats<4, true, true> : k_in_bwd_stats<4, true, false>)
                        : (yb ? k_in_bwd_stats<4, false, true> : k_in_bwd_stats<4, false, false>);
         hipLaunchKernelGGL(kern, grid, dim3(g.threads), sm, s, x, dy, gamma, beta, mean, rstd, partial, C, g.CG, g.R, V,
@@ -668,8 +683,7 @@
         hipLaunchKernelGGL((k_in_bwd_stats<1, false, false>), grid, dim3(g.threads), sm, s, x, dy, gamma, beta, mean, rstd,
                            partial, C, g.CG, g.R, V, g.chunk, slope);
     if (check_launch("instnorm bwd stats")) return 1;
-    hipLaunchKernelGGL(k_in_bwd_finalize, dim3(C), dim3(64), 0, s, partial, sums, dgamma, dbeta, N, C,
-                       g.nblk);
+    hipLaunchKernelGGL(k_in_bwd_finalize, dim3(C), dim3(64), 0, s, partial, sums, dgamma, dbeta, N, C, nblk);
     if (check_launch("instnorm bwd finalize")) return 1;
     long per_n = V * C / (v4 ? 4 : 1);
     long bx = cdiv(per_n, 256);
@@ -702,6 +716,16 @@
                            float slope, void *ws, size_t ws_bytes, void *stream) {
     return in_bwd(x, false, dy, false, gamma, beta, mean, rstd, dx, dgamma, dbeta, N, V, C, slope, ws, ws_bytes, stream);
 }
+
+int mvd_instnorm_lrelu_bwd_prestats(const float *x, const float *dy, const float *tile_sums, long ntiles, const float *gamma,
+                                    const float *beta, const float *mean, const float *rstd, float *dx, float *dgamma,
+                                    float *dbeta, int N, long V, int C, float slope, void *ws, size_t ws_bytes, void *stream) {
+    MVD_REQUIRE(tile_sums && ntiles > 0, "instnorm_bwd_prestats: tile sums required");
+    return in_bwd(x, false, dy, false, gamma, beta, mean, rstd, dx, dgamma, dbeta, N, V, C, slope, ws, ws_bytes, stream, tile_sums,
+                  ntiles);
+}
+
+long mvd_in_bwd_prestats_launches(void) { return g_in_bwd_prestats_launches; }
 
 int mvd_instnorm_lrelu_fwd_prestats(const float *x, const float *tile_stats, long ntiles, const float *gamma,
                                     const float *beta, float *y, float *mean, float *rstd, int N, long V, int C, float eps,
diff --git a/multimodal_mvd_seg_amd/ops.py b/multimodal_mvd_seg_amd/ops.py
--- a/multimodal_mvd_seg_amd/ops.py
+++ b/multimodal_mvd_seg_amd/ops.py
@@ -436,6 +436,33 @@
     return b if (b is not None and tuple(b.shape) == tuple(shape) and b.dtype == dtype and _is_cl3d(b)) else None
 
 
+IN_BWD_PRESTATS = [os.environ.get("MVD_IN_BWD_PRESTATS", "1") != "0"]
+
+
+class _InBwdTag:
+    __slots__ = ("x", "mean", "rstd", "gamma", "beta", "slope", "tiles", "ntiles", "buf")
+
+    def __init__(self, x, mean, rstd, gamma, beta, slope):
+        self.x, self.mean, self.rstd, self.gamma, self.beta, self.slope = x, mean, rstd, gamma, beta, float(slope)
+        self.tiles = self.ntiles = self.buf = None
+
+    def fill(self, tiles, ntiles, buf):
+        self.tiles, self.ntiles, self.buf = tiles, int(ntiles), buf
+
+    def matches(self, dy):
+        return (self.tiles is not None and self.buf is not None and dy.data_ptr() == self.buf.data_ptr()
+                and tuple(dy.shape) == tuple(self.buf.shape) and dy.dtype == self.buf.dtype)
+
+    def release(self):
+        self.x = self.mean = self.rstd = self.gamma = self.beta = self.tiles = self.ntiles = self.buf = None
+
+
+def _in_bwd_tag_for(tag, kind, shape, N, D, H, W, C1):
+    if tag is None or not IN_BWD_PRESTATS[0] or tag.x is None or tuple(tag.x.shape) != tuple(shape):
+        return None
+    return tag if query("mvd_in_bwd_prestats_select", kind, N, D, H, W, C1) else None
+
+
 class LaunchTimer:
 
     def __init__(self, key):
@@ -472,6 +499,8 @@
     def forward(ctx, x1, x2, weight, bias, stride):
         _require_cuda(x1, x2, weight, bias)
         ctx.share1, ctx.share2 = _share_of(x1), (_share_of(x2) if x2 is not None else None)
+        ctx.in_tag1 = getattr(x1, "_mvd_in_bwd", None)
+        ctx.ub3 = False
         x1 = to_ndhwc(x1)
         x2 = to_ndhwc(x2) if x2 is not None else None
         K, C = weight.shape[:2]
@@ -553,7 +582,15 @@
                 call("mvd_conv3d_dgrad_bf16_acc", _p(dy), _p(wb), _p(joined), C1, N, D, H, W, K, i3(ks), i3(stride), _p(ws),
                      ws.numel(), _stream())
             else:
-                call("mvd_conv3d_dgrad_acc", _p(dy), _p(wb), _p(joined), C1, N, D, H, W, K, i3(ks), i3(stride), _stream())
+                tag = None if ctx.bf else _in_bwd_tag_for(ctx.in_tag1, 1, joined.shape, N, D, H, W, C1)
+                if tag is not None:
+                    nt = query("mvd_conv3d_dgrad_acc_sum_tiles", D, H, W)
+                    tiles = torch.empty((N, nt, C1, 2), dtype=torch.float32, device=dev)
+                    call("mvd_conv3d_dgrad_acc_bwdstats", _p(dy), _p(wb), _p(joined), C1, N, D, H, W, K, i3(ks), i3(stride),
+                         _p(tag.x), _p(tag.mean), _p(tag.rstd), _p(tag.gamma), _p(tag.beta), tag.slope, _p(tiles), _stream())
+                    tag.fill(tiles, nt, joined)
+                else:
+                    call("mvd_conv3d_dgrad_acc", _p(dy), _p(wb), _p(joined), C1, N, D, H, W, K, i3(ks), i3(stride), _stream())
             ctx.share1.buf = None
             need1 = False
         elif need1 or need2:
@@ -564,8 +601,20 @@
                 call("mvd_conv3d_dgrad_bf16", _p(dy), _p(wb), _p(dx1), C1, _p(dx2), C2, N, D, H, W, K, i3(ks), i3(stride),
                      _p(ws), ws.numel(), _stream())
             else:
-                call("mvd_conv3d_dgrad_wino3" if ctx.ub3 else "mvd_conv3d_dgrad_wino", _p(dy), _p(wb), _p(ub), _p(dx1), C1,
-                     _p(dx2), C2, N, D, H, W, K, i3(ks), i3(stride), _p(ws), ws.numel(), _stream())
+                tag = _in_bwd_tag_for(ctx.in_tag1, 0, dx1.shape, N, D, H, W, C1) \
+                    if (need1 and x2 is None and ctx.share1 is None and ctx.ub3) else None
+                if tag is not None:
+                    nt = query("mvd_conv_stats_tiles", D, H, W)
+                    tiles = torch.empty((N, nt, C1, 2), dtype=torch.float32, device=dev)
+                    done = ctypes.c_int(0)
+                    call("mvd_conv3d_dgrad_wino3_bwdstats", _p(dy), _p(wb), _p(ub), _p(dx1), C1, None, 0, N, D, H, W, K, i3(ks),
+                         i3(stride), _p(tag.x), _p(tag.mean), _p(tag.rstd), _p(tag.gamma), _p(tag.beta), tag.slope, _p(tiles),
+                         ctypes.byref(done), _p(ws), ws.numel(), _stream())
+                    if done.value:
+                        tag.fill(tiles, nt, dx1)
+                else:
+                    call("mvd_conv3d_dgrad_wino3" if ctx.ub3 else "mvd_conv3d_dgrad_wino", _p(dy), _p(wb), _p(ub), _p(dx1),
+                         C1, _p(dx2), C2, N, D, H, W, K, i3(ks), i3(stride), _p(ws), ws.numel(), _stream())
             if need1:
                 _publish(ctx.share1, dx1)
             if need2:
@@ -778,6 +827,9 @@
         ctx.slope = float(slope)
         ctx.yb = yb
         ctx.params = (gamma, beta)
+        ctx.bwd_tag = None
+        if not yb and IN_BWD_PRESTATS[0] and C % 32 == 0:
+            ctx.bwd_tag = y._mvd_in_bwd = _InBwdTag(x, mean, rstd, g, b, slope)
         return y
 
     @staticmethod
@@ -795,12 +847,18 @@
         db = sink_b if sink_b is not None else torch.empty((C,), dtype=torch.float32, device=x.device)
         nb = query("mvd_instnorm_workspace_bytes", N, V, C)
         ws = _Workspace.get(nb, x.device)
+        tag = ctx.bwd_tag
         if ctx.yb:
             call("mvd_instnorm_lrelu_bwd_bf16", _p(x), int(_is_bf16(x)), _p(dy), _p(g), _p(b), _p(mean), _p(rstd), _p(dx),
                  _p(dg), _p(db), N, V, C, ctx.slope, _p(ws), ws.numel(), _stream())
+        elif tag is not None and tag.matches(dy):
+            call("mvd_instnorm_lrelu_bwd_prestats", _p(x), _p(dy), _p(tag.tiles), tag.ntiles, _p(g), _p(b), _p(mean), _p(rstd),
+                 _p(dx), _p(dg), _p(db), N, V, C, ctx.slope, _p(ws), ws.numel(), _stream())
         else:
             call("mvd_instnorm_lrelu_bwd", _p(x), _p(dy), _p(g), _p(b), _p(mean), _p(rstd), _p(dx), _p(dg), _p(db), N, V,
                  C, ctx.slope, _p(ws), ws.numel(), _stream())
+        if tag is not None:
+            tag.release()
         if sink_g is not None:
             dg = None
             _grad_done(gamma)
```

Measured after the change: 60.66 samples/s (median of 6 runs). Within noise of the previous version (+0.3%).
